# cwchenwang/outdoor-nerf-depth

Hardware: AMD Instinct MI355X
Metric: train rays/sec, KITTI 375x1242, 64+128 samples/ray (higher is better)
Workload: dtype bf16 MFMA operands, f32 accumulate / f32 master weights

## Files before the change

include/nerfpp_hip.h:

```cpp
#ifndef NERFPP_HIP_H
#define NERFPP_HIP_H

#include <stdint.h>

#ifdef __cplusplus
extern "C" {
#endif

#define NERFPP_ABI_VERSION 9

#define NERFPP_OK 0
#define NERFPP_ERR_ARG 1
#define NERFPP_ERR_HIP 2
#define NERFPP_ERR_INTERNAL 3
#define NERFPP_ERR_UNSUPPORTED 4
#define NERFPP_ERR_COMM 5
#define NERFPP_ERR_LAUNCH NERFPP_ERR_HIP

#define NERFPP_PREC_BF16 1
#define NERFPP_PREC_SPLIT_BF16 2
#define NERFPP_PREC_FP16X2W 3

#define NERFPP_LOSS_RGB_ONLY 0
#define NERFPP_LOSS_MSE 1
#define NERFPP_LOSS_L1 2
#define NERFPP_LOSS_KL 3

#define NERFPP_FG_PARAMS 595844
#define NERFPP_BG_PARAMS 606596
#define NERFPP_LEVEL_PARAMS 1202440
#define NERFPP_MAX_SAMPLES 256

const char* nerfpp_last_error(void);
int nerfpp_abi_version(void);


int nerfpp_intersect_sphere(void* stream, int n_rays, const float* ray_o, const float* ray_d,
                            float* fg_far, int* bad_count);

int nerfpp_sample_coarse(void* stream, int n_rays, int n_samples, const float* ray_o,
                         const float* ray_d, const float* min_depth, const float* t_rand_fg,
                         const float* t_rand_bg, float* fg_far, float* fg_z, float* bg_z,
                         int* bad_count);

int nerfpp_sample_coarse_rng(void* stream, int n_rays, int n_samples, const float* ray_o,
                             const float* ray_d, const float* min_depth, uint64_t seed, uint64_t step,
                             float* fg_far, float* fg_z, float* bg_z, int* bad_count);

int nerfpp_rng_uniform(void* stream, uint64_t seed, uint64_t step, int stream_id, int64_t n, float* out);

int nerfpp_perturb_samples(void* stream, int n_rays, int n_samples, const float* z_vals,
                           const float* t_rand, float* out);

int nerfpp_sample_pdf(void* stream, int n_rays, int n_bins_m, int n_new, const float* bins,
                      const float* weights, const float* u, float* samples, int64_t* above_inds);

int nerfpp_sample_fine(void* stream, int n_rays, int s_old, int n_new, const float* z_old,
                       const float* weights, const float* u, float* z_merged, float* samples,
                       int64_t* above_inds);

int nerfpp_sample_fine_pair(void* stream, int n_rays, int s_old, int n_new, const float* fg_z_old,
                            const float* fg_weights, const float* fg_u, float* fg_z_merged,
                            const float* bg_z_old, const float* bg_weights, const float* bg_u,
                            float* bg_z_merged);

int nerfpp_sample_fine_pair_rng(void* stream, int n_rays, int s_old, int n_new, const float* fg_z_old,
                                const float* fg_weights, float* fg_z_merged, const float* bg_z_old,
                                const float* bg_weights, float* bg_z_merged, uint64_t seed, uint64_t step);

int nerfpp_sample_pixels(void* stream, uint64_t seed, uint64_t step, int64_t n_pixels, int n_rays, int64_t* pix);

int nerfpp_gather_rays(void* stream, int n_rays, int width, const float* cam, const int64_t* pix,
                       const float* rgb_img, const float* depth_img, float* ray_o, float* ray_d,
                       float* rgb, float* depth_sup, float* min_depth);


int nerfpp_table_sizes(int net, int64_t* fwd_elems, int64_t* fwd_bias_elems, int64_t* bwd_elems,
                       int64_t* slab_floats, int64_t* n_params);
int nerfpp_build_tables(int net, int32_t* fwd_tbl, int32_t* bias_tbl, int32_t* bwd_tbl,
                        int32_t* unpack_tbl);
int64_t nerfpp_level_tables_elems(void);
int nerfpp_build_level_tables(int32_t* host_tables);

int nerfpp_dw_plan(int64_t rows, int backward_precision, int32_t* k_out, int32_t* is_full_out);

int64_t nerfpp_packed_bytes(int precision);
int nerfpp_pack_level(void* stream, int precision, const float* params, const int32_t* tables,
                      void* packed);


int64_t nerfpp_workspace_bytes(int n_rays, int n_samples, int precision, int training);

int nerfpp_workspace_tensor(int n_rays, int n_samples, int precision, int net, int tensor,
                            int64_t* byte_offset, int32_t* ld, int64_t* plane_bytes);

typedef struct {
  int32_t n_rays, n_samples;
  int32_t precision, training;
  const float* ray_o;
  const float* ray_d;
  const float* fg_far;
  const float* fg_z;
  const float* bg_z;
  const void* packed;
  void* workspace;
  float* rgb;
  float* depth;
  float* fg_weights;
  float* bg_weights;
  float* fg_dists;
  float* fg_rgb;
  float* fg_depth;
  float* bg_rgb;
  float* bg_depth;
  float* bg_lambda;
  void* ev_mlp_begin;
  void* ev_mlp_end;
} nerfpp_forward_args;

int nerfpp_level_forward(void* stream, const nerfpp_forward_args* args);

int nerfpp_loss(void* stream, int n_rays, int n_samples, int loss_type, float lambda_depth,
                float kl_sigma, const float* rgb, const float* rgb_gt, const float* depth,
                const float* depth_sup, const float* fg_weights, const float* fg_z,
                const float* fg_dists, const float* fg_far, float* scalars, float* g_rgb,
                float* g_depth, float* g_fg_weights);

typedef struct {
  int32_t n_rays, n_samples;
  int32_t precision;
  int32_t workspace_precision;
  const float* ray_d;
  const float* fg_far;
  const float* fg_z;
  const float* bg_z;
  const void* packed;
  void* workspace;
  const int32_t* tables;
  const float* g_rgb;
  const float* g_depth;
  const float* g_fg_weights;
  float grad_scale;
  float* grads;
  void* ev_bwd_begin;
  void* ev_bwd_end;
  void* ev_dw_begin;
  void* ev_dw_end;
  const float* params;
  int32_t defer_reduce;
  int32_t fused_loss;
  int32_t loss_type;
  float lambda_depth;
  float kl_sigma;
  const float* rgb;
  const float* depth;
  const float* rgb_gt;
  const float* depth_sup;
  const int32_t* bad_count;
} nerfpp_backward_args;

int nerfpp_level_backward(void* stream, const nerfpp_backward_args* args);

int nerfpp_level_reduce_grads(void* stream, const nerfpp_backward_args* args);

int nerfpp_adam_step(void* stream, float* params, const float* grads, float* exp_avg,
                     float* exp_avg_sq, int64_t n, int step, double lr, double beta1, double beta2,
                     double eps, const float* skip_if_nonzero);

const char* nerfpp_comm_last_error(void);
int nerfpp_rccl_unique_id(char out_id[128]);
int nerfpp_rccl_comm_init(void** comm, int world_size, const char id[128], int rank);
int nerfpp_rccl_comm_destroy(void* comm);
int nerfpp_allreduce_mean(void* stream, void* rccl_comm, float* grads, int64_t count, int world_size, int prescaled);

int64_t nerfpp_image_metrics_workspace_bytes(int n_frames, int H, int W);
int nerfpp_image_metrics_u8(void* stream, int n_frames, int H, int W, const uint8_t* gt, const uint8_t* pred,
                            void* workspace, double* out);

#ifdef __cplusplus
}
#endif
#endif
```

outdoor_nerf_depth_amd/_lib.py:

```python
import ctypes as C
import os

from . import _ctypes_util as U

_HERE = os.path.dirname(os.path.abspath(__file__))
LIB_PATH = os.environ.get('NERFPP_HIP_LIB') or os.path.join(_HERE, 'libnerfpp_hip.so')

OK = 0
ABI_VERSION = 9
PREC_BF16, PREC_SPLIT_BF16 = 1, 2
PREC_FP16_FWD = 3
PREC_SPLIT_FWD = 12
LOSS_RGB_ONLY, LOSS_MSE, LOSS_L1, LOSS_KL = 0, 1, 2, 3
LOSS_TYPES = {'rgbonly': LOSS_RGB_ONLY, 'mse': LOSS_MSE, 'l1': LOSS_L1, 'kl': LOSS_KL}
FG_PARAMS, BG_PARAMS, LEVEL_PARAMS = 595844, 606596, 1202440
MAX_SAMPLES = 256

_fp = C.c_void_p
_i64p = C.POINTER(C.c_int64)
_i32p = C.POINTER(C.c_int32)


class ForwardArgs(C.Structure):
    _fields_ = [('n_rays', C.c_int32), ('n_samples', C.c_int32), ('precision', C.c_int32),
                ('training', C.c_int32)] + \
               [(k, _fp) for k in ('ray_o', 'ray_d', 'fg_far', 'fg_z', 'bg_z', 'packed', 'workspace',
                                   'rgb', 'depth', 'fg_weights', 'bg_weights', 'fg_dists', 'fg_rgb',
                                   'fg_depth', 'bg_rgb', 'bg_depth', 'bg_lambda', 'ev_mlp_begin',
                                   'ev_mlp_end')]


class BackwardArgs(C.Structure):
    _fields_ = [('n_rays', C.c_int32), ('n_samples', C.c_int32), ('precision', C.c_int32),
                ('workspace_precision', C.c_int32)] + \
               [(k, _fp) for k in ('ray_d', 'fg_far', 'fg_z', 'bg_z', 'packed', 'workspace', 'tables',
                                   'g_rgb', 'g_depth', 'g_fg_weights')] + \
               [('grad_scale', C.c_float), ('grads', _fp)] + \
               [(k, _fp) for k in ('ev_bwd_begin', 'ev_bwd_end', 'ev_dw_begin', 'ev_dw_end', 'params')] + \
               [('defer_reduce', C.c_int32), ('fused_loss', C.c_int32), ('loss_type', C.c_int32),
                ('lambda_depth', C.c_float), ('kl_sigma', C.c_float)] + \
               [(k, _fp) for k in ('rgb', 'depth', 'rgb_gt', 'depth_sup', 'bad_count')]


SYMBOLS = {
    'nerfpp_last_error': (C.c_char_p, []),
    'nerfpp_abi_version': (C.c_int, []),
    'nerfpp_intersect_sphere': (C.c_int, [_fp, C.c_int, _fp, _fp, _fp, _fp]),
    'nerfpp_sample_coarse': (C.c_int, [_fp, C.c_int, C.c_int] + [_fp] * 9),
    'nerfpp_sample_coarse_rng': (C.c_int, [_fp, C.c_int, C.c_int, _fp, _fp, _fp, C.c_uint64, C.c_uint64, _fp, _fp, _fp, _fp]),
    'nerfpp_rng_uniform': (C.c_int, [_fp, C.c_uint64, C.c_uint64, C.c_int, C.c_int64, _fp]),
    'nerfpp_sample_pixels': (C.c_int, [_fp, C.c_uint64, C.c_uint64, C.c_int64, C.c_int, _fp]),
    'nerfpp_perturb_samples': (C.c_int, [_fp, C.c_int, C.c_int, _fp, _fp, _fp]),
    'nerfpp_sample_pdf': (C.c_int, [_fp, C.c_int, C.c_int, C.c_int, _fp, _fp, _fp, _fp, _fp]),
    'nerfpp_sample_fine': (C.c_int, [_fp, C.c_int, C.c_int, C.c_int, _fp, _fp, _fp, _fp, _fp, _fp]),
    'nerfpp_sample_fine_pair': (C.c_int, [_fp, C.c_int, C.c_int, C.c_int, _fp, _fp, _fp, _fp, _fp, _fp, _fp, _fp]),
    'nerfpp_sample_fine_pair_rng': (C.c_int, [_fp, C.c_int, C.c_int, C.c_int, _fp, _fp, _fp, _fp, _fp, _fp, C.c_uint64,
                                              C.c_uint64]),
    'nerfpp_gather_rays': (C.c_int, [_fp, C.c_int, C.c_int] + [_fp] * 9),
    'nerfpp_table_sizes': (C.c_int, [C.c_int, _i64p, _i64p, _i64p, _i64p, _i64p]),
    'nerfpp_build_tables': (C.c_int, [C.c_int, _i32p, _i32p, _i32p, _i32p]),
    'nerfpp_level_tables_elems': (C.c_int64, []),
    'nerfpp_build_level_tables': (C.c_int, [_i32p]),
    'nerfpp_dw_plan': (C.c_int, [C.c_int64, C.c_int, _i32p, _i32p]),
    'nerfpp_packed_bytes': (C.c_int64, [C.c_int]),
    'nerfpp_pack_level': (C.c_int, [_fp, C.c_int, _fp, _fp, _fp]),
    'nerfpp_workspace_bytes': (C.c_int64, [C.c_int, C.c_int, C.c_int, C.c_int]),
    'nerfpp_workspace_tensor': (C.c_int, [C.c_int, C.c_int, C.c_int, C.c_int, C.c_int, _i64p, _i32p, _i64p]),
    'nerfpp_level_forward': (C.c_int, [_fp, C.POINTER(ForwardArgs)]),
    'nerfpp_loss': (C.c_int, [_fp, C.c_int, C.c_int, C.c_int, C.c_float, C.c_float] + [_fp] * 12),
    'nerfpp_level_backward': (C.c_int, [_fp, C.POINTER(BackwardArgs)]),
    'nerfpp_level_reduce_grads': (C.c_int, [_fp, C.POINTER(BackwardArgs)]),
    'nerfpp_adam_step': (C.c_int, [_fp, _fp, _fp, _fp, _fp, C.c_int64, C.c_int, C.c_double, C.c_double,
                                   C.c_double, C.c_double, _fp]),
    'nerfpp_image_metrics_workspace_bytes': (C.c_int64, [C.c_int, C.c_int, C.c_int]),
    'nerfpp_image_metrics_u8': (C.c_int, [_fp, C.c_int, C.c_int, C.c_int, _fp, _fp, _fp, _fp]),
    'nerfpp_comm_last_error': (C.c_char_p, []),
    'nerfpp_rccl_unique_id': (C.c_int, [C.c_char_p]),
    'nerfpp_rccl_comm_init': (C.c_int, [C.POINTER(C.c_void_p), C.c_int, C.c_char_p, C.c_int]),
    'nerfpp_rccl_comm_destroy': (C.c_int, [_fp]),
    'nerfpp_allreduce_mean': (C.c_int, [_fp, _fp, _fp, C.c_int64, C.c_int, C.c_int]),
}

_lib = None


class NerfppError(RuntimeError):
    pass


def lib():
    global _lib
    if _lib is None:
        _lib = U.load(LIB_PATH, 'libnerfpp_hip.so', SYMBOLS, 'nerfpp_abi_version', ABI_VERSION, NerfppError,
                      ' (hipcc --offload-arch=gfx950). There is no CPU fallback for the NeRF++ hot path.')
    return _lib


check = U.checker(lib, 'nerfpp_last_error', NerfppError, 'nerfpp call')


def build_level_tables():
    import numpy as np
    n = lib().nerfpp_level_tables_elems()
    out = np.empty(n, np.int32)
    check(lib().nerfpp_build_level_tables(out.ctypes.data_as(_i32p)), 'nerfpp_build_level_tables')
    return out


def build_net_tables(net):
    import numpy as np
    sizes = [C.c_int64() for _ in range(5)]
    check(lib().nerfpp_table_sizes(net, *[C.byref(s) for s in sizes]), 'nerfpp_table_sizes')
    fwd, bias, bwd, slab, npar = [s.value for s in sizes]
    arrs = [np.empty(n, np.int32) for n in (fwd, bias, bwd, npar)]
    check(lib().nerfpp_build_tables(net, *[a.ctypes.data_as(_i32p) for a in arrs]), 'nerfpp_build_tables')
    return arrs[0], arrs[1], arrs[2], arrs[3], slab
```

outdoor_nerf_depth_amd/csrc/nerfpp_api.hip:

```cpp
#include "probe_env.h"
#include <hip/hip_runtime.h>
#include <stdio.h>
#include <stdlib.h>
#include <string.h>
#include "../../include/nerfpp_hip.h"
#define API_OK NERFPP_OK
#define API_ERR_HIP NERFPP_ERR_HIP
#define API_ERR_ARG NERFPP_ERR_ARG
#include "api_common.h"
#include "nerfpp_common.h"
#include "nerfpp_kernels.h"

using namespace nerfpp;

namespace {

constexpr size_t align_up(size_t v, size_t a) { return (v + a - 1) / a * a; }
bool h0_recomputed(int WP) { return a_planes(WP) == 1; }

struct TblLayout { int64_t fwd[2], bias[2], bwd[2], unpack[2], total; };
TblLayout tbl_layout() {
  TblLayout L{};
  int64_t off = 0;
  for (int net = 0; net < N_NET; ++net) {
    L.fwd[net] = off; off += (int64_t)fwd_frags(net) * 512;
    L.bias[net] = off; off += FWD_BIAS_FLOATS;
    L.bwd[net] = off; off += (int64_t)BWD_FRAGS * 512;
    L.unpack[net] = off; off += net_params(net);
  }
  L.total = off;
  return L;
}

struct PackLayout { size_t fwd[2], bwd[2], bias[2], derived[2], total; };
PackLayout pack_layout(int P) {
  PackLayout L{};
  size_t off = 0;
  for (int net = 0; net < N_NET; ++net) {
    L.fwd[net] = off; off = align_up(off + fwd_stream_bytes(net, P), 256);
    L.bwd[net] = off; off = align_up(off + bwd_stream_bytes(P), 256);
    L.bias[net] = off; off = align_up(off + FWD_BIAS_FLOATS * sizeof(float), 256);
    L.derived[net] = off; off = align_up(off + DERIVED_FLOATS * sizeof(float), 256);
  }
  L.total = off;
  return L;
}

struct WsLayout {
  size_t tensor[2][T_COUNT], out_raw[2], depth_real, d_out[2], slabs[2], masks[2], fix_m[2], total;
  int64_t rows, rows_padded;
  int ksplit;
};
int choose_ksplit(int64_t rows) {
  int k = 1;
  for (int rc = 0; rc < 2; ++rc) {
    const DwPlan pl = dw_plan(rows, rc != 0);
    for (int net = 0; net < N_NET; ++net)
      for (int j = 0; j < DW_JOBS; ++j) k = pl.k[net][j] > k ? pl.k[net][j] : k;
  }
  return k;
}
WsLayout ws_layout(int n_rays, int S, int P, bool training) {
  WsLayout L{};
  L.rows = (int64_t)n_rays * S;
  L.rows_padded = (int64_t)align_up((size_t)L.rows, 256);
  L.ksplit = choose_ksplit(L.rows);
  size_t off = 0;
  for (int net = 0; net < N_NET; ++net) {
    L.out_raw[net] = off; off = align_up(off + (size_t)L.rows_padded * 16, 256);
    if (training) {
      L.d_out[net] = off; off = align_up(off + (size_t)L.rows_padded * 16, 256);
      for (int t = 0; t < T_COUNT; ++t) {
        L.tensor[net][t] = off;
        if (t == T_R || t == T_DR) continue;
        if (t == T_DG) continue;
        if (t == T_H0 && h0_recomputed(P)) continue;
        if (t == T_DZ0 + 7 && h0_recomputed(P)) continue;
        off = align_up(off + (size_t)L.rows_padded * tensor_ld(net, t) * 2 * a_planes(P), 256);
      }
      L.slabs[net] = off; off = align_up(off + (size_t)L.ksplit * gslab_floats(net) * 4, 256);
      L.masks[net] = off; off = align_up(off + (size_t)9 * (L.rows_padded / 32) * 64 * 16, 256);
      L.fix_m[net] = off; off = align_up(off + (size_t)128 * 256 * 4, 256);
    }
  }
  L.depth_real = off; off = align_up(off + (size_t)L.rows_padded * 4, 256);
  L.total = off;
  return L;
}

NetWs make_netws(char* ws, const WsLayout& L, int net) {
  NetWs w;
  for (int t = 0; t < T_COUNT; ++t) w.t[t] = (__bf16*)(ws + L.tensor[net][t]);
  w.t[T_DG] = w.t[T_DS] + (DG_COL0 / 16) * (FRAG_BYTES / 2);
  return w;
}

bool prec_ok(int P) { return P == NERFPP_PREC_BF16 || P == NERFPP_PREC_SPLIT_BF16; }
bool prec_ok_fwd(int P) { return prec_ok(P) || P == NERFPP_PREC_FP16X2W; }

bool split_nets() {
  static const bool on = PROBE_GETENV("NERFPP_MLP_SPLIT") != nullptr;
  return on;
}

}

extern "C" {

const char* nerfpp_last_error(void) { return g_err; }
int nerfpp_abi_version(void) { return NERFPP_ABI_VERSION; }

int nerfpp_intersect_sphere(void* stream, int n_rays, const float* ray_o, const float* ray_d, float* fg_far,
                            int* bad_count) {
  REQUIRE(n_rays > 0 && ray_o && ray_d && fg_far, "non-null inputs, n_rays > 0");
  launch_intersect_sphere((hipStream_t)stream, n_rays, ray_o, ray_d, fg_far, bad_count);
  return check_launch("intersect_sphere");
}

int nerfpp_sample_coarse(void* stream, int n_rays, int n_samples, const float* ray_o, const float* ray_d,
                         const float* min_depth, const float* t_rand_fg, const float* t_rand_bg, float* fg_far,
                         float* fg_z, float* bg_z, int* bad_count) {
  REQUIRE(n_rays > 0 && n_samples >= 2 && n_samples <= NERFPP_MAX_SAMPLES, "2 <= n_samples <= 256");
  REQUIRE(ray_o && ray_d && min_depth && fg_far && fg_z && bg_z, "non-null pointers");
  launch_sample_coarse((hipStream_t)stream, n_rays, n_samples, ray_o, ray_d, min_depth, t_rand_fg, t_rand_bg,
                       fg_far, fg_z, bg_z, bad_count, make_rng_key(0, 0, false));
  return check_launch("sample_coarse");
}

int nerfpp_sample_coarse_rng(void* stream, int n_rays, int n_samples, const float* ray_o, const float* ray_d,
                             const float* min_depth, uint64_t seed, uint64_t step, float* fg_far, float* fg_z,
                             float* bg_z, int* bad_count) {
  REQUIRE(n_rays > 0 && n_samples >= 2 && n_samples <= NERFPP_MAX_SAMPLES, "2 <= n_samples <= 256");
  REQUIRE(ray_o && ray_d && min_depth && fg_far && fg_z && bg_z, "non-null pointers");
  launch_sample_coarse((hipStream_t)stream, n_rays, n_samples, ray_o, ray_d, min_depth, nullptr, nullptr, fg_far,
                       fg_z, bg_z, bad_count, make_rng_key(seed, step, true));
  return check_launch("sample_coarse_rng");
}

int nerfpp_rng_uniform(void* stream, uint64_t seed, uint64_t step, int stream_id, int64_t n, float* out) {
  REQUIRE(n > 0 && out && stream_id >= 0 && stream_id <= 3, "stream_id in 0..3, non-null output");
  launch_rng_uniform((hipStream_t)stream, make_rng_key(seed, step, true), (uint32_t)stream_id, n, out);
  return check_launch("rng_uniform");
}

int nerfpp_perturb_samples(void* stream, int n_rays, int n_samples, const float* z_vals, const float* t_rand,
                           float* out) {
  REQUIRE(n_rays > 0 && n_samples >= 2 && z_vals && t_rand && out, "non-null pointers");
  launch_perturb((hipStream_t)stream, n_rays, n_samples, z_vals, t_rand, out);
  return check_launch("perturb_samples");
}

int nerfpp_sample_pdf(void* stream, int n_rays, int n_bins_m, int n_new, const float* bins, const float* weights,
                      const float* u, float* samples, int64_t* above_inds) {
  REQUIRE(n_rays > 0 && n_bins_m >= 1 && n_bins_m + 1 <= 512 && n_new >= 1 && n_new <= 512, "sizes");
  REQUIRE(bins && weights && samples, "non-null pointers");
  launch_sample_pdf((hipStream_t)stream, false, n_rays, n_bins_m, n_new, bins, weights, u, samples, above_inds,
                    nullptr);
  return check_launch("sample_pdf");
}

int nerfpp_sample_fine(void* stream, int n_rays, int s_old, int n_new, const float* z_old, const float* weights,
                       const float* u, float* z_merged, float* samples, int64_t* above_inds) {
  REQUIRE(n_rays > 0 && s_old >= 3 && n_new >= 1 && s_old + n_new <= 512, "3 <= s_old, s_old + n_new <= 512");
  REQUIRE(z_old && weights && z_merged, "non-null pointers");
  launch_sample_pdf((hipStream_t)stream, true, n_rays, s_old - 2, n_new, z_old, weights, u, samples, above_inds,
                    z_merged);
  return check_launch("sample_fine");
}

int nerfpp_sample_fine_pair(void* stream, int n_rays, int s_old, int n_new, const float* fg_z_old,
                            const float* fg_weights, const float* fg_u, float* fg_z_merged, const float* bg_z_old,
                            const float* bg_weights, const float* bg_u, float* bg_z_merged) {
  REQUIRE(n_rays > 0 && s_old >= 3 && n_new >= 1 && s_old + n_new <= 512, "3 <= s_old, s_old + n_new <= 512");
  REQUIRE(fg_z_old && fg_weights && fg_z_merged && bg_z_old && bg_weights && bg_z_merged, "non-null pointers");
  const float* z[2] = {fg_z_old, bg_z_old};
  const float* w[2] = {fg_weights, bg_weights};
  const float* u[2] = {fg_u, bg_u};
  float* m[2] = {fg_z_merged, bg_z_merged};
  launch_sample_fine_pair((hipStream_t)stream, n_rays, s_old - 2, n_new, z, w, u, m, make_rng_key(0, 0, false));
  return check_launch("sample_fine_pair");
}

int nerfpp_sample_fine_pair_rng(void* stream, int n_rays, int s_old, int n_new, const float* fg_z_old,
                                const float* fg_weights, float* fg_z_merged, const float* bg_z_old,
                                const float* bg_weights, float* bg_z_merged, uint64_t seed, uint64_t step) {
  REQUIRE(n_rays > 0 && s_old >= 3 && n_new >= 1 && s_old + n_new <= 512, "3 <= s_old, s_old + n_new <= 512");
  REQUIRE(fg_z_old && fg_weights && fg_z_merged && bg_z_old && bg_weights && bg_z_merged, "non-null pointers");
  const float* z[2] = {fg_z_old, bg_z_old};
  const float* w[2] = {fg_weights, bg_weights};
  const float* u[2] = {nullptr, nullptr};
  float* m[2] = {fg_z_merged, bg_z_merged};
  launch_sample_fine_pair((hipStream_t)stream, n_rays, s_old - 2, n_new, z, w, u, m, make_rng_key(seed, step, true));
  return check_launch("sample_fine_pair_rng");
}

int nerfpp_sample_pixels(void* stream, uint64_t seed, uint64_t step, int64_t n_pixels, int n_rays, int64_t* pix) {
  REQUIRE(pix && n_rays >= 1 && n_rays <= 8192, "1 <= n_rays <= 8192, non-null output");
  REQUIRE(n_pixels >= n_rays && n_pixels < ((int64_t)1 << 31), "n_rays <= n_pixels < 2^31");
  launch_sample_pixels((hipStream_t)stream, make_rng_key(seed, step, true), n_pixels, n_rays, pix);
  return check_launch("sample_pixels");
}

int nerfpp_gather_rays(void* stream, int n_rays, int width, const float* cam, const int64_t* pix,
                       const float* rgb_img, const float* depth_img, float* ray_o, float* ray_d, float* rgb,
                       float* depth_sup, float* min_depth) {
  REQUIRE(n_rays > 0 && width > 0 && cam && pix && ray_o && ray_d && min_depth, "non-null pointers");
  REQUIRE((rgb == nullptr) || rgb_img, "rgb output needs rgb_img");
  REQUIRE((depth_sup == nullptr) || depth_img, "depth_sup output needs depth_img");
  launch_gather_rays((hipStream_t)stream, n_rays, width, cam, pix, rgb_img, depth_img, ray_o, ray_d, rgb, depth_sup,
                     min_depth);
  return check_launch("gather_rays");
}

int64_t nerfpp_level_tables_elems(void) { return tbl_layout().total; }

int nerfpp_build_level_tables(int32_t* host_tables) {
  if (!host_tables) return fail(NERFPP_ERR_ARG, "nerfpp_build_level_tables: null buffer");
  const TblLayout L = tbl_layout();
  for (int net = 0; net < N_NET; ++net) {
    const int rc = nerfpp_build_tables(net, host_tables + L.fwd[net], host_tables + L.bias[net],
                                       host_tables + L.bwd[net], host_tables + L.unpack[net]);
    if (rc != NERFPP_OK) return fail(rc, "nerfpp_build_tables(%d) failed", net);
  }
  return NERFPP_OK;
}

int nerfpp_dw_plan(int64_t rows, int backward_precision, int32_t* k_out, int32_t* is_full_out) {
  if (!k_out || rows <= 0 || !prec_ok(backward_precision)) return -1;
  const DwPlan pl = dw_plan(rows, backward_precision == 1);
  const JobTable jt = build_all_jobs();
  for (int net = 0; net < N_NET; ++net)
    for (int j = 0; j < DW_JOBS; ++j) {
      k_out[net * DW_JOBS + j] = pl.k[net][j];
      if (is_full_out) is_full_out[net * DW_JOBS + j] = dw_job_is_full(jt.jobs[net][j]) ? 1 : 0;
    }
  return DW_JOBS;
}

int64_t nerfpp_packed_bytes(int precision) { return prec_ok_fwd(precision) ? (int64_t)pack_layout(precision).total : -1; }

int nerfpp_pack_level(void* stream, int precision, const float* params, const int32_t* tables, void* packed) {
  REQUIRE(prec_ok_fwd(precision), "precision must be 1, 2 or 3");
  REQUIRE(params && tables && packed, "non-null pointers");
  const TblLayout T = tbl_layout();
  const PackLayout L = pack_layout(precision);
  hipStream_t st = (hipStream_t)stream;
  char* out = (char*)packed;
  const int32_t* tbl[3 * N_NET];
  void* outs[3 * N_NET];
  int64_t n[3 * N_NET];
  for (int net = 0; net < N_NET; ++net) {
    tbl[3 * net] = tables + T.fwd[net];      outs[3 * net] = out + L.fwd[net];      n[3 * net] = (int64_t)fwd_frags(net) * 512;
    tbl[3 * net + 1] = tables + T.bwd[net];  outs[3 * net + 1] = out + L.bwd[net];  n[3 * net + 1] = (int64_t)BWD_FRAGS * 512;
    tbl[3 * net + 2] = tables + T.bias[net]; outs[3 * net + 2] = out + L.bias[net]; n[3 * net + 2] = FWD_BIAS_FLOATS;
  }
  float* derived[N_NET] = {(float*)(out + L.derived[0]), (float*)(out + L.derived[1])};
  launch_pack_level(st, params, precision, tbl, outs, n, derived);
  return check_launch("pack_level");
}

int64_t nerfpp_workspace_bytes(int n_rays, int n_samples, int precision, int training) {
  if (n_rays <= 0 || n_samples < 2 || n_samples > NERFPP_MAX_SAMPLES || !prec_ok_fwd(precision)) return -1;
  return (int64_t)ws_layout(n_rays, n_samples, precision, training != 0).total;
}

int nerfpp_workspace_tensor(int n_rays, int n_samples, int precision, int net, int tensor, int64_t* byte_offset,
                            int32_t* ld, int64_t* plane_bytes) {
  REQUIRE(n_rays > 0 && n_samples >= 2 && n_samples <= NERFPP_MAX_SAMPLES && prec_ok_fwd(precision), "sizes / precision");
  REQUIRE(net >= 0 && net < N_NET && tensor >= 0 && tensor < T_COUNT && tensor != T_R && tensor != T_DR, "net / tensor id");
  REQUIRE(byte_offset && ld && plane_bytes, "non-null outputs");
  if (tensor == T_H0 && h0_recomputed(precision))
    return fail(NERFPP_ERR_UNSUPPORTED, "nerfpp_workspace_tensor: H0 is not materialised at precision %d (its weight-gradient job recomputes it from X)", precision);
  if (tensor == T_DZ0 + 7 && h0_recomputed(precision))
    return fail(NERFPP_ERR_UNSUPPORTED, "nerfpp_workspace_tensor: dZ7 is not materialised at precision %d (its weight-gradient job recomputes it from [dS | dG])", precision);
  const WsLayout L = ws_layout(n_rays, n_samples, precision, true);
  const int l = tensor_ld(net, tensor);
  *byte_offset = tensor == T_DG ? (int64_t)L.tensor[net][T_DS] + (DG_COL0 / 16) * FRAG_BYTES : (int64_t)L.tensor[net][tensor];
  *ld = l;
  *plane_bytes = (int64_t)L.rows_padded * l * 2;
  return NERFPP_OK;
}

int nerfpp_level_forward(void* stream, const nerfpp_forward_args* a) {
  REQUIRE(a, "args");
  REQUIRE(a->n_rays > 0 && a->n_samples >= 2 && a->n_samples <= NERFPP_MAX_SAMPLES, "sizes");
  REQUIRE(prec_ok_fwd(a->precision), "precision must be 1, 2 or 3");
  REQUIRE(a->ray_o && a->ray_d && a->fg_far && a->fg_z && a->bg_z && a->packed && a->workspace, "inputs");
  REQUIRE(a->rgb && a->depth && a->fg_weights && a->bg_weights && a->fg_dists && a->fg_rgb && a->fg_depth &&
          a->bg_rgb && a->bg_depth && a->bg_lambda, "outputs");
  hipStream_t st = (hipStream_t)stream;
  const int P = a->precision;
  const bool train = a->training != 0;
  const WsLayout L = ws_layout(a->n_rays, a->n_samples, P, train);
  const PackLayout PL = pack_layout(P);
  char* ws = (char*)a->workspace;
  const char* pk = (const char*)a->packed;
  MlpFwdArgs mm[N_NET];
  for (int net = 0; net < N_NET; ++net) {
    MlpFwdArgs& m = mm[net];
    m = MlpFwdArgs{};
    m.geom.ray_o = a->ray_o;
    m.geom.ray_d = a->ray_d;
    m.geom.z = net == 0 ? a->fg_z : a->bg_z;
    m.rows = L.rows;
    m.rows_padded = L.rows_padded;
    m.S = a->n_samples;
    m.w_stream = pk + PL.fwd[net];
    m.bias = (const float*)(pk + PL.bias[net]);
    m.out_raw = (float*)(ws + L.out_raw[net]);
    m.depth_real = (float*)(ws + L.depth_real);
    if (train) { m.ws = make_netws(ws, L, net); m.masks = (uint4*)(ws + L.masks[net]); }
    m.save_lo = a->training == 2 ? 0 : 1;
    m.skip_h0 = (train && (h0_recomputed(P) || a->training == 2)) ? 1 : 0;
    if (const char* e = PROBE_GETENV("NERFPP_SKIP_H_RT")) m.save_lo |= atoi(e) << 8;
  }
  if (a->ev_mlp_begin) (void)hipEventRecord((hipEvent_t)a->ev_mlp_begin, st);
  if (split_nets()) {
    launch_mlp_fwd_pair(st, P, train, mm[0], mm[1], 1);
    launch_mlp_fwd_pair(st, P, train, mm[0], mm[1], 2);
  } else {
    launch_mlp_fwd_pair(st, P, train, mm[0], mm[1], 0);
  }
  if (a->ev_mlp_end) (void)hipEventRecord((hipEvent_t)a->ev_mlp_end, st);
  launch_composite_fwd(st, a->n_rays, a->n_samples, (const float*)(ws + L.out_raw[0]),
                       (const float*)(ws + L.out_raw[1]), (const float*)(ws + L.depth_real), a->ray_d, a->fg_far,
                       a->fg_z, a->bg_z, a->rgb, a->depth, a->fg_weights, a->bg_weights, a->fg_dists, a->fg_rgb,
                       a->fg_depth, a->bg_rgb, a->bg_depth, a->bg_lambda);
  return check_launch("level_forward");
}

int nerfpp_loss(void* stream, int n_rays, int n_samples, int loss_type, float lambda_depth, float kl_sigma,
                const float* rgb, const float* rgb_gt, const float* depth, const float* depth_sup,
                const float* fg_weights, const float* fg_z, const float* fg_dists, const float* fg_far,
                float* scalars, float* g_rgb, float* g_depth, float* g_fg_weights) {
  REQUIRE(n_rays > 0 && loss_type >= 0 && loss_type <= 3, "loss_type in 0..3");
  REQUIRE(rgb && rgb_gt && scalars && g_rgb && g_depth, "non-null pointers");
  if (loss_type != NERFPP_LOSS_RGB_ONLY) REQUIRE(depth && depth_sup, "depth loss needs depth and depth_sup");
  if (loss_type == NERFPP_LOSS_KL)
    REQUIRE(fg_weights && fg_z && fg_dists && fg_far && g_fg_weights && kl_sigma > 0.f, "KL inputs");
  launch_loss((hipStream_t)stream, n_rays, n_samples, loss_type, lambda_depth, kl_sigma, rgb, rgb_gt, depth,
              depth_sup, fg_weights, fg_z, fg_dists, fg_far, scalars, g_rgb, g_depth, g_fg_weights);
  return check_launch("loss");
}

}

static void weight_grads(hipStream_t st, const nerfpp_backward_args* a, const WsLayout& L) {
  char* ws = (char*)a->workspace;
  DwArgs dw{};
  for (int net = 0; net < N_NET; ++net) {
    dw.ws[net] = make_netws(ws, L, net);
    dw.slabs[net] = (float*)(ws + L.slabs[net]);
  }
  dw.rows = L.rows;
  dw.rows_padded = L.rows_padded;
  dw.h0_from_x = a->precision == 1 ? 1 : 0;
  const PackLayout PL = pack_layout(a->precision);
  for (int net = 0; net < N_NET; ++net) {
    dw.fwd_w[net] = (const char*)a->packed + PL.fwd[net];
    dw.fwd_bias[net] = (const float*)((const char*)a->packed + PL.bias[net]);
    dw.bwd_w[net] = (const char*)a->packed + PL.bwd[net];
    dw.masks[net] = (const uint4*)(ws + L.masks[net]);
  }
  dw.plan = dw_plan(L.rows, dw.h0_from_x != 0);
  if (a->ev_dw_begin) (void)hipEventRecord((hipEvent_t)a->ev_dw_begin, st);
  launch_dw(st, a->precision, dw);
  if (a->ev_dw_end) (void)hipEventRecord((hipEvent_t)a->ev_dw_end, st);
}
static bool defer_dw() {
  static const bool on = PROBE_GETENV("NERFPP_DEFER_DW") != nullptr;
  return on;
}

static void reduce_grads(hipStream_t st, const nerfpp_backward_args* a, const WsLayout& L, const TblLayout& T) {
  char* ws = (char*)a->workspace;
  const DwPlan plan = dw_plan(L.rows, a->precision == 1);
  const float* slabs[N_NET];
  int64_t slab_floats[N_NET];
  const int32_t* utbl[N_NET];
  float* m_out[N_NET];
  for (int net = 0; net < N_NET; ++net) {
    slabs[net] = (const float*)(ws + L.slabs[net]);
    slab_floats[net] = gslab_floats(net);
    utbl[net] = a->tables + T.unpack[net];
    m_out[net] = (float*)(ws + L.fix_m[net]);
  }
  static const int skip = PROBE_GETENV("NERFPP_REDUCE_SKIP") ? atoi(PROBE_GETENV("NERFPP_REDUCE_SKIP")) : 0;
  if (!(skip & 1)) launch_unpack_grads(st, slabs, slab_floats, plan, utbl, m_out, a->grad_scale, a->grads, a->bad_count);
  if (!(skip & 2)) launch_remap_fixup(st, a->grads, a->params, m_out[0], m_out[1]);
}

extern "C" {

int nerfpp_level_reduce_grads(void* stream, const nerfpp_backward_args* a) {
  REQUIRE(a, "args");
  REQUIRE(a->n_rays > 0 && a->n_samples >= 2 && a->n_samples <= NERFPP_MAX_SAMPLES, "sizes");
  REQUIRE(prec_ok(a->precision), "precision must be 1 or 2");
  REQUIRE(a->workspace && a->tables && a->grads && a->params, "workspace / tables / grads / params");
  const int WP = a->workspace_precision ? a->workspace_precision : a->precision;
  REQUIRE(prec_ok_fwd(WP) && a_planes(WP) >= a_planes(a->precision), "workspace_precision: 0, or a forward precision that saved the planes this backward reads");
  const WsLayout L = ws_layout(a->n_rays, a->n_samples, WP, true);
  if (defer_dw()) weight_grads((hipStream_t)stream, a, L);
  reduce_grads((hipStream_t)stream, a, L, tbl_layout());
  return check_launch("level_reduce_grads");
}

int nerfpp_level_backward(void* stream, const nerfpp_backward_args* a) {
  REQUIRE(a, "args");
  REQUIRE(a->n_rays > 0 && a->n_samples >= 2 && a->n_samples <= NERFPP_MAX_SAMPLES, "sizes");
  REQUIRE(prec_ok(a->precision), "precision must be 1 or 2");
  REQUIRE(a->ray_d && a->fg_far && a->fg_z && a->bg_z && a->packed && a->workspace && a->tables, "inputs");
  REQUIRE(a->grads && a->params, "gradients / params");
  LossFuse lf{};
  if (a->fused_loss) {
    REQUIRE(a->loss_type >= NERFPP_LOSS_RGB_ONLY && a->loss_type <= NERFPP_LOSS_KL, "loss_type in 0..3");
    REQUIRE(a->rgb && a->rgb_gt, "fused loss head needs rgb and rgb_gt");
    if (a->loss_type != NERFPP_LOSS_RGB_ONLY) REQUIRE(a->depth && a->depth_sup, "fused depth loss needs depth and depth_sup");
    if (a->loss_type == NERFPP_LOSS_KL) REQUIRE(a->kl_sigma > 0.f, "kl_sigma > 0");
    lf.type = a->loss_type; lf.lambda_depth = a->lambda_depth; lf.kl_sigma = a->kl_sigma;
    lf.rgb = a->rgb; lf.depth = a->depth; lf.rgb_gt = a->rgb_gt; lf.depth_sup = a->depth_sup;
  } else {
    REQUIRE(a->g_rgb && a->g_depth, "dL/d rgb and dL/d depth (or fused_loss)");
  }
  hipStream_t st = (hipStream_t)stream;
  const int P = a->precision;
  const int WP = a->workspace_precision ? a->workspace_precision : P;
  REQUIRE(prec_ok_fwd(WP) && a_planes(WP) >= a_planes(P), "workspace_precision: 0, or a forward precision that saved the planes this backward reads");
  const WsLayout L = ws_layout(a->n_rays, a->n_samples, WP, true);
  const PackLayout PL = pack_layout(P);
  const TblLayout T = tbl_layout();
  char* ws = (char*)a->workspace;
  const char* pk = (const char*)a->packed;
  launch_composite_bwd(st, a->n_rays, a->n_samples, (const float*)(ws + L.out_raw[0]),
                       (const float*)(ws + L.out_raw[1]), (const float*)(ws + L.depth_real), a->ray_d, a->fg_far,
                       a->fg_z, a->bg_z, a->g_rgb, a->g_depth, a->g_fg_weights, (float*)(ws + L.d_out[0]),
                       (float*)(ws + L.d_out[1]), a->fused_loss ? &lf : nullptr);
  MlpBwdArgs mb[N_NET];
  for (int net = 0; net < N_NET; ++net) {
    MlpBwdArgs& m = mb[net];
    m = MlpBwdArgs{};
    m.rows = L.rows;
    m.rows_padded = L.rows_padded;
    m.w_stream = pk + PL.bwd[net];
    m.d_out = (const float*)(ws + L.d_out[net]);
    m.ws = make_netws(ws, L, net);
    m.masks = (const uint4*)(ws + L.masks[net]);
    m.skip_dz7 = P == 1 ? 1 : 0;
  }
  if (a->ev_bwd_begin) (void)hipEventRecord((hipEvent_t)a->ev_bwd_begin, st);
  if (split_nets()) {
    launch_mlp_bwd_pair(st, P, mb[0], mb[1], 1);
    launch_mlp_bwd_pair(st, P, mb[0], mb[1], 2);
  } else {
    launch_mlp_bwd_pair(st, P, mb[0], mb[1], 0);
  }
  if (a->ev_bwd_end) (void)hipEventRecord((hipEvent_t)a->ev_bwd_end, st);
  if (!(a->defer_reduce && defer_dw())) weight_grads(st, a, L);
  if (!a->defer_reduce) reduce_grads(st, a, L, T);
  return check_launch("level_backward");
}

int nerfpp_adam_step(void* stream, float* params, const float* grads, float* exp_avg, float* exp_avg_sq,
                     int64_t n, int step, double lr, double beta1, double beta2, double eps,
                     const float* skip_if_nonzero) {
  REQUIRE(params && grads && exp_avg && exp_avg_sq && n > 0 && step >= 1, "non-null pointers, step >= 1");
  launch_adam((hipStream_t)stream, params, grads, exp_avg, exp_avg_sq, n, step, lr, beta1, beta2, eps, skip_if_nonzero);
  return check_launch("adam_step");
}

static int image_metrics_sizes_ok(const char* fn, int n_frames, int H, int W) {
  if (n_frames < 1 || n_frames > 65535) return fail(NERFPP_ERR_ARG, "%s: n_frames = %d, expected 1 .. 65535", fn, n_frames);
  if (H < 7 || W < 7)
    return fail(NERFPP_ERR_ARG, "%s: a %d x %d image is smaller than the 7 x 7 SSIM window (H >= 7 and W >= 7)", fn, H, W);
  if (H > 32768 || W > 32768) return fail(NERFPP_ERR_ARG, "%s: a %d x %d image exceeds 32768 pixels per side", fn, H, W);
  return NERFPP_OK;
}

int64_t nerfpp_image_metrics_workspace_bytes(int n_frames, int H, int W) {
  if (image_metrics_sizes_ok(__func__, n_frames, H, W) != NERFPP_OK) return -1;
  return (int64_t)n_frames * image_metrics_tiles(H, W) * 4 * 8;
}

int nerfpp_image_metrics_u8(void* stream, int n_frames, int H, int W, const uint8_t* gt, const uint8_t* pred,
                            void* workspace, double* out) {
  const int rc = image_metrics_sizes_ok(__func__, n_frames, H, W);
  if (rc != NERFPP_OK) return rc;
  REQUIRE(gt && pred && workspace && out, "non-null gt, pred, workspace, out");
  REQUIRE(((uintptr_t)workspace & 7) == 0 && ((uintptr_t)out & 7) == 0, "workspace and out aligned to 8 bytes");
  launch_image_metrics((hipStream_t)stream, n_frames, H, W, gt, pred, workspace, out);
  return check_launch("image_metrics_u8");
}

}
```

outdoor_nerf_depth_amd/csrc/nerfpp_kernels.h:

```cpp
#pragma once
#include <hip/hip_runtime.h>
#include <stdint.h>
#include "nerfpp_common.h"

namespace nerfpp {

struct MlpGeom {
  const float* ray_o;
  const float* ray_d;
  const float* z;
};

struct NetWs {
  __bf16* t[T_COUNT];
};

struct MlpFwdArgs {
  MlpGeom geom;
  int64_t rows, rows_padded;
  int S;
  const void* w_stream;
  const float* bias;
  float* out_raw;
  float* depth_real;
  NetWs ws;
  uint4* masks;
  int save_lo;
  int skip_h0;
};

struct MlpBwdArgs {
  int64_t rows, rows_padded;
  const void* w_stream;
  const float* d_out;
  NetWs ws;
  const uint4* masks;
  int skip_dz7;
};

struct LossFuse {
  int type;
  float lambda_depth, kl_sigma;
  const float* rgb;
  const float* depth;
  const float* rgb_gt;
  const float* depth_sup;
};

struct DwArgs {
  NetWs ws[N_NET];
  int64_t rows, rows_padded;
  float* slabs[N_NET];
  DwPlan plan;
  int h0_from_x;
  const void* fwd_w[N_NET];
  const float* fwd_bias[N_NET];
  const void* bwd_w[N_NET];
  const uint4* masks[N_NET];
};

}

void launch_intersect_sphere(hipStream_t st, int n, const float* o, const float* d, float* far, int* bad);
void launch_sample_coarse(hipStream_t st, int n, int S, const float* o, const float* d, const float* min_depth,
                          const float* t_fg, const float* t_bg, float* far, float* fg_z, float* bg_z, int* bad,
                          const nerfpp::RngKey& rng);
void launch_rng_uniform(hipStream_t st, const nerfpp::RngKey& rng, uint32_t stream_id, int64_t n, float* out);
void launch_perturb(hipStream_t st, int n, int S, const float* z, const float* t, float* out);
void launch_sample_pdf(hipStream_t st, bool fused, int n, int M, int S_new, const float* bins_or_zold,
                       const float* weights, const float* u, float* samples, int64_t* above, float* merged);
void launch_sample_fine_pair(hipStream_t st, int n, int M, int S_new, const float* const* z_old,
                             const float* const* weights, const float* const* u, float* const* merged,
                             const nerfpp::RngKey& rng);
void launch_composite_fwd(hipStream_t st, int n, int S, const float* raw_fg, const float* raw_bg,
                          const float* depth_real_bg, const float* ray_d, const float* fg_far,
                          const float* fg_z, const float* bg_z, float* rgb, float* depth, float* fg_weights,
                          float* bg_weights, float* fg_dists, float* fg_rgb, float* fg_depth, float* bg_rgb,
                          float* bg_depth, float* bg_lambda);
void launch_composite_bwd(hipStream_t st, int n, int S, const float* raw_fg, const float* raw_bg,
                          const float* depth_real_bg, const float* ray_d, const float* fg_far,
                          const float* fg_z, const float* bg_z, const float* g_rgb, const float* g_depth,
                          const float* g_fg_weights, float* dout_fg, float* dout_bg, const nerfpp::LossFuse* lf);
void launch_loss(hipStream_t st, int n, int S, int type, float lambda_depth, float kl_sigma, const float* rgb,
                 const float* rgb_gt, const float* depth, const float* depth_sup, const float* fg_weights,
                 const float* fg_z, const float* fg_dists, const float* fg_far, float* scalars, float* g_rgb,
                 float* g_depth, float* g_fg_weights);
int launch_sample_pixels(hipStream_t st, const nerfpp::RngKey& rng, int64_t n_pixels, int k, int64_t* pix);
void launch_gather_rays(hipStream_t st, int n, int W, const float* cam, const int64_t* pix, const float* rgb_img,
                        const float* depth_img, float* ray_o, float* ray_d, float* rgb, float* depth_sup,
                        float* min_depth);
void launch_mlp_fwd_pair(hipStream_t st, int P, bool train, const nerfpp::MlpFwdArgs& a_fg, const nerfpp::MlpFwdArgs& a_bg, int which);
void launch_mlp_bwd_pair(hipStream_t st, int P, const nerfpp::MlpBwdArgs& a_fg, const nerfpp::MlpBwdArgs& a_bg, int which);
void launch_dw(hipStream_t st, int P, const nerfpp::DwArgs& a);
void launch_pack_level(hipStream_t st, const float* params, int P, const int32_t* const* tbl, void* const* out,
                       const int64_t* n, float* const* derived);
void launch_unpack_grads(hipStream_t st, const float* const* slabs, const int64_t* slab_floats,
                         const nerfpp::DwPlan& plan, const int32_t* const* tbl, float* const* m_out, float scale,
                         float* grads_lvl, const int32_t* bad_count);
void launch_remap_fixup(hipStream_t st, float* grads_lvl, const float* params_lvl, const float* m0, const float* m1);
void launch_adam(hipStream_t st, float* p, const float* g, float* m, float* v, int64_t n, int step, double lr,
                 double beta1, double beta2, double eps, const float* skip);
int64_t image_metrics_tiles(int H, int W);
void launch_image_metrics(hipStream_t st, int F, int H, int W, const unsigned char* gt, const unsigned char* pred,
                          void* workspace, double* out);
```

outdoor_nerf_depth_amd/csrc/nerfpp_render.hip:

```cpp
#include <hip/hip_runtime.h>
#include <math.h>
#include <stdint.h>
#include "hip_device.h"
#include "nerfpp_common.h"
#include "nerfpp_kernels.h"

namespace nerfpp {

using hipdev::wave_sum, hipdev::wave_excl_suffix_sum;

constexpr float TINY = 1e-6f;
constexpr float HUGE_NUM = 1e10f;

__device__ __forceinline__ float sum3(float a, float b, float c) { return (a + b) + c; }

__device__ __forceinline__ float sphere_far(const float* __restrict__ ray_o,
                                            const float* __restrict__ ray_d, int ray, int* bad) {
  const float ox = ray_o[ray * 3], oy = ray_o[ray * 3 + 1], oz = ray_o[ray * 3 + 2];
  const float dx = ray_d[ray * 3], dy = ray_d[ray * 3 + 1], dz = ray_d[ray * 3 + 2];
  const float dd = sum3(dx * dx, dy * dy, dz * dz);
  const float d1 = -sum3(dx * ox, dy * oy, dz * oz) / dd;
  const float px = ox + d1 * dx, py = oy + d1 * dy, pz = oz + d1 * dz;
  const float ray_d_cos = 1.f / sqrtf(dd);
  const float pn = sum3(px * px, py * py, pz * pz);
  if (pn >= 1.f && bad) atomicAdd(bad, 1);
  const float d2 = sqrtf(1.f - pn) * ray_d_cos;
  return d1 + d2;
}

__global__ void intersect_sphere_kernel(int n, const float* __restrict__ ray_o,
                                        const float* __restrict__ ray_d, float* __restrict__ far,
                                        int* bad) {
  const int ray = blockIdx.x * blockDim.x + threadIdx.x;
  if (ray < n) far[ray] = sphere_far(ray_o, ray_d, ray, bad);
}

__device__ __forceinline__ float torch_linspace01(int i, int steps) {
  const float step = 1.f / (float)(steps - 1);
  return i < steps / 2 ? fmaf(step, (float)i, 0.f) : fmaf(-step, (float)(steps - 1 - i), 1.f);
}

__device__ __forceinline__ float perturb(float zm, float z0, float zp, bool first, bool last, float t) {
  const float upper = last ? z0 : .5f * (zp + z0);
  const float lower = first ? z0 : .5f * (z0 + zm);
  return lower + (upper - lower) * t;
}

__global__ void sample_coarse_kernel(int n, int S, const float* __restrict__ ray_o,
                                     const float* __restrict__ ray_d,
                                     const float* __restrict__ min_depth,
                                     const float* __restrict__ t_fg, const float* __restrict__ t_bg,
                                     float* __restrict__ fg_far, float* __restrict__ fg_z,
                                     float* __restrict__ bg_z, int* bad, RngKey rng) {
  const int idx = blockIdx.x * blockDim.x + threadIdx.x;
  if (idx >= n * S) return;
  const int ray = idx / S, i = idx - ray * S;
  const float far = sphere_far(ray_o, ray_d, ray, i == 0 ? bad : nullptr);
  if (i == 0) fg_far[ray] = far;
  const float near = min_depth[ray];
  const float step = (far - near) / (float)(S - 1);
  const float z0 = near + (float)i * step;
  float out = z0;
  if (t_fg || rng.enabled) {
    const float zm = near + (float)(i - 1) * step, zp = near + (float)(i + 1) * step;
    out = perturb(zm, z0, zp, i == 0, i == S - 1, rng.enabled ? philox_uniform(rng, 0, (uint64_t)idx) : t_fg[idx]);
  }
  fg_z[idx] = out;
  const float b0 = torch_linspace01(i, S);
  out = b0;
  if (t_bg || rng.enabled) {
    const float bm = i > 0 ? torch_linspace01(i - 1, S) : 0.f;
    const float bp = i < S - 1 ? torch_linspace01(i + 1, S) : 0.f;
    out = perturb(bm, b0, bp, i == 0, i == S - 1, rng.enabled ? philox_uniform(rng, 1, (uint64_t)idx) : t_bg[idx]);
  }
  bg_z[idx] = out;
}

__global__ void rng_uniform_kernel(RngKey rng, uint32_t stream_id, int64_t n, float* __restrict__ out) {
  const int64_t i = (int64_t)blockIdx.x * blockDim.x + threadIdx.x;
  if (i < n) out[i] = philox_uniform(rng, stream_id, (uint64_t)i);
}

__global__ void perturb_kernel(int n, int S, const float* __restrict__ z, const float* __restrict__ t,
                               float* __restrict__ out) {
  const int idx = blockIdx.x * blockDim.x + threadIdx.x;
  if (idx >= n * S) return;
  const int i = idx % S;
  const float z0 = z[idx];
  const float zm = i > 0 ? z[idx - 1] : 0.f, zp = i < S - 1 ? z[idx + 1] : 0.f;
  out[idx] = perturb(zm, z0, zp, i == 0, i == S - 1, t[idx]);
}

constexpr int SP_MAX = 512;
__device__ __forceinline__ void lds_wave_sync() {
  asm volatile("s_waitcnt lgkmcnt(0)" ::: "memory");
  __builtin_amdgcn_wave_barrier();
}

struct SamplePdfProblem {
  const float* bins_or_zold; const float* weights; const float* u;
  float* samples; int64_t* above; float* merged;
};
struct SamplePdfArgs { SamplePdfProblem p[2]; RngKey rng; };
template <bool FUSED>
__global__ __launch_bounds__(256) void sample_pdf_kernel(int n, int M, int S_new, SamplePdfArgs args) {
  const SamplePdfProblem& pr = args.p[blockIdx.y];
  const float* __restrict__ bins_or_zold = pr.bins_or_zold;
  const float* __restrict__ weights = pr.weights;
  const float* __restrict__ u_in = pr.u;
  float* __restrict__ samples_out = pr.samples;
  int64_t* __restrict__ above_out = pr.above;
  float* __restrict__ merged_out = pr.merged;
  __shared__ float s_cdf[4][SP_MAX];
  __shared__ float s_w[4][SP_MAX];
  __shared__ float s_bins[4][SP_MAX];
  __shared__ float s_z[4][SP_MAX];
  const int wave = threadIdx.x >> 6, lane = threadIdx.x & 63;
  const int ray = blockIdx.x * 4 + wave;
  const bool active = ray < n;
  const int S_old = FUSED ? M + 2 : 0;
  float* cdf = s_cdf[wave];
  float* wq = s_w[wave];
  float* bins = s_bins[wave];
  float* zs = s_z[wave];
  if (active) {
    if (FUSED) {
      const float* zo = bins_or_zold + (size_t)ray * S_old;
      for (int i = lane; i < S_old; i += 64) zs[i] = zo[i];
      for (int k = lane; k < M; k += 64) wq[k] = weights[(size_t)ray * S_old + k + 1] + TINY;
    } else {
      for (int i = lane; i <= M; i += 64) bins[i] = bins_or_zold[(size_t)ray * (M + 1) + i];
      for (int k = lane; k < M; k += 64) wq[k] = weights[(size_t)ray * M + k] + TINY;
    }
  }
  __syncthreads();
  if (active) {
    if (FUSED)
      for (int i = lane; i <= M; i += 64) bins[i] = .5f * (zs[i + 1] + zs[i]);
    if (lane == 0) {
      double acc = 0.0;
      for (int k = 0; k < M; ++k) acc += (double)wq[k];
      cdf[0] = (float)acc;
    }
  }
  __syncthreads();
  if (active) {
    const float wsum = cdf[0];
    for (int k = lane; k < M; k += 64) wq[k] = wq[k] / wsum;
  }
  __syncthreads();
  if (active && lane == 0) {
    double acc = 0.0;
    cdf[0] = 0.f;
    for (int k = 0; k < M; ++k) {
      acc += (double)wq[k];
      cdf[k + 1] = (float)acc;
    }
  }
  __syncthreads();
  if (active) {
    for (int j = lane; j < S_new; j += 64) {
      const float u = args.rng.enabled ? philox_uniform(args.rng, 2u + blockIdx.y, (uint64_t)ray * S_new + j)
                      : u_in ? u_in[(size_t)ray * S_new + j] : torch_linspace01(j, S_new);
      int above = 0, hi_ = M;
      while (above < hi_) {
        const int mid = (above + hi_) >> 1;
        const bool ge = u >= cdf[mid];
        above = ge ? mid + 1 : above;
        hi_ = ge ? hi_ : mid;
      }
      const int below = above - 1 > 0 ? above - 1 : 0;
      const float cdf_lo = cdf[below], cdf_hi = cdf[above];
      const float bin_lo = bins[below], bin_hi = bins[above];
      float denom = cdf_hi - cdf_lo;
      denom = denom < TINY ? 1.f : denom;
      const float t = (u - cdf_lo) / denom;
      const float s = bin_lo + t * (bin_hi - bin_lo + TINY);
      if (samples_out) samples_out[(size_t)ray * S_new + j] = s;
      if (above_out) above_out[(size_t)ray * S_new + j] = above;
      if (FUSED) zs[S_old + j] = s;
    }
  }
  if (!FUSED) return;
  __syncthreads();
  if (active && merged_out) {
    const int S_tot = S_old + S_new;
    bool sorted_old = true;
    for (int i = lane; i + 1 < S_old; i += 64) sorted_old = sorted_old && zs[i] <= zs[i + 1];
    if (__all(sorted_old) && S_new <= SP_MAX) {
      int P2 = 1;
      while (P2 < S_new) P2 <<= 1;
      float* nb = wq;
      for (int i = lane; i < P2; i += 64) nb[i] = i < S_new ? zs[S_old + i] : __builtin_inff();
      lds_wave_sync();
      for (int k = 2; k <= P2; k <<= 1) {
        for (int j = k >> 1; j > 0; j >>= 1) {
          for (int t = lane; t < (P2 >> 1); t += 64) {
            const int lo = ((t & ~(j - 1)) << 1) | (t & (j - 1)), hi_i = lo | j;
            const bool up = (lo & k) == 0;
            const float x = nb[lo], y = nb[hi_i];
            if ((x > y) == up) { nb[lo] = y; nb[hi_i] = x; }
          }
          lds_wave_sync();
        }
      }
      float* mo = merged_out + (size_t)ray * S_tot;
      for (int i = lane; i < S_old; i += 64) {
        const float v = zs[i];
        int lo = 0, hi_i = S_new;
        while (lo < hi_i) {
          const int mid = (lo + hi_i) >> 1;
          const bool lt = nb[mid] < v;
          lo = lt ? mid + 1 : lo;
          hi_i = lt ? hi_i : mid;
        }
        mo[i + lo] = v;
      }
      for (int p = lane; p < S_new; p += 64) {
        const float v = nb[p];
        int lo = 0, hi_i = S_old;
        while (lo < hi_i) {
          const int mid = (lo + hi_i) >> 1;
          const bool le = zs[mid] <= v;
          lo = le ? mid + 1 : lo;
          hi_i = le ? hi_i : mid;
        }
        mo[p + lo] = v;
      }
      return;
    }
    if (S_tot <= 192) {
      const int e0 = lane, e1 = lane + 64, e2 = lane + 128;
      const float v0 = e0 < S_tot ? zs[e0] : 0.f, v1 = e1 < S_tot ? zs[e1] : 0.f, v2 = e2 < S_tot ? zs[e2] : 0.f;
      int r0 = 0, r1 = 0, r2 = 0;
#pragma unroll 4
      for (int k = 0; k < S_tot; ++k) {
        const float o = zs[k];
        r0 += (o < v0 || (o == v0 && k < e0)) ? 1 : 0;
        r1 += (o < v1 || (o == v1 && k < e1)) ? 1 : 0;
        r2 += (o < v2 || (o == v2 && k < e2)) ? 1 : 0;
      }
      float* mo = merged_out + (size_t)ray * S_tot;
      if (e0 < S_tot) mo[r0] = v0;
      if (e1 < S_tot) mo[r1] = v1;
      if (e2 < S_tot) mo[r2] = v2;
      return;
    }
    for (int e = lane; e < S_tot; e += 64) {
      const float v = zs[e];
      int rank = 0;
      for (int k = 0; k < S_tot; ++k) {
        const float o = zs[k];
        rank += (o < v || (o == v && k < e)) ? 1 : 0;
      }
      merged_out[(size_t)ray * S_tot + rank] = v;
    }
  }
}

constexpr int CPL_MAX = 4;

__device__ __forceinline__ float wave_excl_prod(float x, int lane, float* total) {
  float v = x;
#pragma unroll
  for (int d = 1; d < 64; d <<= 1) {
    const float t = __shfl_up(v, d, 64);
    if (lane >= d) v *= t;
  }
  *total = __shfl(v, 63, 64);
  const float e = __shfl_up(v, 1, 64);
  return lane == 0 ? 1.f : e;
}

struct RaySamples {
  float dist[CPL_MAX], e[CPL_MAX], alpha[CPL_MAX], q[CPL_MAX], T[CPL_MAX], w[CPL_MAX];
  float c[CPL_MAX][3], zval[CPL_MAX], sraw[CPL_MAX];
  float lambda;
};

template <bool BG>
__device__ __forceinline__ void load_volume(RaySamples& v, int S, int cpl, int lane, size_t row0,
                                            const float4* __restrict__ raw, const float* __restrict__ z,
                                            const float* __restrict__ depth_real, float dnorm, float far) {
  float run = 1.f;
#pragma unroll
  for (int k = 0; k < CPL_MAX; ++k) {
    const int i = lane * cpl + k;
    const bool ok = k < cpl && i < S;
    float dist = 0.f, sraw = 0.f, zv = 0.f;
    float c0 = 0.f, c1 = 0.f, c2 = 0.f;
    if (ok) {
      const int s = BG ? S - 1 - i : i;
      const float4 r = raw[row0 + s];
      c0 = r.x; c1 = r.y; c2 = r.z; sraw = r.w;
      if (BG) {
        const float zi = z[s];
        dist = i < S - 1 ? zi - z[s - 1] : HUGE_NUM;
        zv = depth_real[row0 + s];
      } else {
        const float zi = z[i];
        dist = dnorm * ((i < S - 1 ? z[i + 1] : far) - zi);
        zv = zi;
      }
    }
    const float sigma = fabsf(sraw);
    const float e = ok ? expf(-sigma * dist) : 1.f;
    const float alpha = 1.f - e;
    const float q = ok ? 1.f - alpha + TINY : 1.f;
    v.dist[k] = dist; v.e[k] = e; v.alpha[k] = alpha; v.q[k] = q;
    v.c[k][0] = c0; v.c[k][1] = c1; v.c[k][2] = c2; v.zval[k] = zv; v.sraw[k] = sraw;
    v.T[k] = run;
    run *= q;
  }
  float total;
  const float pre = wave_excl_prod(run, lane, &total);
  v.lambda = total;
#pragma unroll
  for (int k = 0; k < CPL_MAX; ++k) {
    v.T[k] *= pre;
    v.w[k] = v.alpha[k] * v.T[k];
  }
}

__global__ __launch_bounds__(256) void composite_fwd_kernel(
    int n, int S, const float4* __restrict__ raw_fg, const float4* __restrict__ raw_bg,
    const float* __restrict__ depth_real_bg, const float* __restrict__ ray_d,
    const float* __restrict__ fg_far, const float* __restrict__ fg_z, const float* __restrict__ bg_z,
    float* __restrict__ rgb, float* __restrict__ depth, float* __restrict__ fg_weights,
    float* __restrict__ bg_weights, float* __restrict__ fg_dists, float* __restrict__ fg_rgb,
    float* __restrict__ fg_depth, float* __restrict__ bg_rgb, float* __restrict__ bg_depth,
    float* __restrict__ bg_lambda) {
  const int wave = threadIdx.x >> 6, lane = threadIdx.x & 63;
  const int ray = blockIdx.x * 4 + wave;
  if (ray >= n) return;
  const int cpl = (S + 63) / 64;
  const size_t row0 = (size_t)ray * S;
  const float dx = ray_d[ray * 3], dy = ray_d[ray * 3 + 1], dz = ray_d[ray * 3 + 2];
  const float dnorm = sqrtf(sum3(dx * dx, dy * dy, dz * dz));
  RaySamples v;
  load_volume<false>(v, S, cpl, lane, row0, raw_fg, fg_z + row0, nullptr, dnorm, fg_far[ray]);
  float a0 = 0, a1 = 0, a2 = 0, ad = 0;
#pragma unroll
  for (int k = 0; k < CPL_MAX; ++k) {
    const int i = lane * cpl + k;
    if (k < cpl && i < S) {
      fg_weights[row0 + i] = v.w[k];
      fg_dists[row0 + i] = v.dist[k];
      a0 += v.w[k] * v.c[k][0]; a1 += v.w[k] * v.c[k][1]; a2 += v.w[k] * v.c[k][2];
      ad += v.w[k] * v.zval[k];
    }
  }
  const float f0 = wave_sum(a0), f1 = wave_sum(a1), f2 = wave_sum(a2), fd = wave_sum(ad);
  const float lam = v.lambda;
  load_volume<true>(v, S, cpl, lane, row0, raw_bg, bg_z + row0, depth_real_bg, dnorm, 0.f);
  a0 = a1 = a2 = ad = 0;
#pragma unroll
  for (int k = 0; k < CPL_MAX; ++k) {
    const int i = lane * cpl + k;
    if (k < cpl && i < S) {
      bg_weights[row0 + i] = v.w[k];
      a0 += v.w[k] * v.c[k][0]; a1 += v.w[k] * v.c[k][1]; a2 += v.w[k] * v.c[k][2];
      ad += v.w[k] * v.zval[k];
    }
  }
  const float b0 = lam * wave_sum(a0), b1 = lam * wave_sum(a1), b2 = lam * wave_sum(a2);
  const float bd = lam * wave_sum(ad);
  if (lane == 0) {
    fg_rgb[ray * 3] = f0; fg_rgb[ray * 3 + 1] = f1; fg_rgb[ray * 3 + 2] = f2;
    bg_rgb[ray * 3] = b0; bg_rgb[ray * 3 + 1] = b1; bg_rgb[ray * 3 + 2] = b2;
    rgb[ray * 3] = f0 + b0; rgb[ray * 3 + 1] = f1 + b1; rgb[ray * 3 + 2] = f2 + b2;
    fg_depth[ray] = fd; bg_depth[ray] = bd; depth[ray] = fd + bd; bg_lambda[ray] = lam;
  }
}

struct KlFuse { bool on; float gt, inv2s, lambda_depth; };
template <bool BG>
__device__ __forceinline__ void volume_backward(const RaySamples& v, int S, int cpl, int lane, size_t row0,
                                                const float gC[3], float gD, float g_lam_lam,
                                                const float* __restrict__ g_w_extra,
                                                float4* __restrict__ dout, const KlFuse kl = KlFuse{false, 0.f, 0.f, 0.f}) {
  float gw[CPL_MAX], term = 0.f;
#pragma unroll
  for (int k = 0; k < CPL_MAX; ++k) {
    const int i = lane * cpl + k;
    const bool ok = k < cpl && i < S;
    float g = gC[0] * v.c[k][0] + gC[1] * v.c[k][1] + gC[2] * v.c[k][2] + gD * v.zval[k];
    if (ok && g_w_extra) g += g_w_extra[row0 + i];
    if (!BG && ok && kl.on) {
      const float dz = v.zval[k] - kl.gt;
      const float w = v.w[k] + 1e-5f;
      const float e = expf(-(dz * dz) * kl.inv2s);
      g += -kl.lambda_depth * e * v.dist[k] / (w * (float)S);
    }
    gw[k] = ok ? g : 0.f;
    term += gw[k] * v.w[k];
  }
  float suffix = wave_excl_suffix_sum(term, lane);
#pragma unroll
  for (int k = CPL_MAX - 1; k >= 0; --k) {
    const int i = lane * cpl + k;
    if (k < cpl && i < S) {
      const float d_a = gw[k] * v.T[k] - (suffix + g_lam_lam) / v.q[k];
      const float d_sigma = d_a * v.dist[k] * v.e[k];
      const float sgn = v.sraw[k] > 0.f ? 1.f : (v.sraw[k] < 0.f ? -1.f : 0.f);
      float4 o;
      o.x = v.w[k] * gC[0] * v.c[k][0] * (1.f - v.c[k][0]);
      o.y = v.w[k] * gC[1] * v.c[k][1] * (1.f - v.c[k][1]);
      o.z = v.w[k] * gC[2] * v.c[k][2] * (1.f - v.c[k][2]);
      o.w = d_sigma * sgn;
      const int s = BG ? S - 1 - i : i;
      dout[row0 + s] = o;
    }
    suffix += gw[k] * v.w[k];
  }
}

template <bool LF>
__global__ __launch_bounds__(256) void composite_bwd_kernel(
    int n, int S, const float4* __restrict__ raw_fg, const float4* __restrict__ raw_bg,
    const float* __restrict__ depth_real_bg, const float* __restrict__ ray_d,
    const float* __restrict__ fg_far, const float* __restrict__ fg_z, const float* __restrict__ bg_z,
    const float* __restrict__ g_rgb, const float* __restrict__ g_depth,
    const float* __restrict__ g_fg_weights, float4* __restrict__ dout_fg, float4* __restrict__ dout_bg, LossFuse lf) {
  const int wave = threadIdx.x >> 6, lane = threadIdx.x & 63;
  const int ray = blockIdx.x * 4 + wave;
  float cnt = 0.f;
  if (LF && (lf.type == 1 || lf.type == 2)) {
    __shared__ float s_cnt[4];
    float c = 0.f;
    for (int r = threadIdx.x; r < n; r += 256) c += lf.depth_sup[r] > 0.f ? 1.f : 0.f;
    c = wave_sum(c);
    if (lane == 0) s_cnt[wave] = c;
    __syncthreads();
    cnt = (s_cnt[0] + s_cnt[1]) + (s_cnt[2] + s_cnt[3]);
  }
  if (ray >= n) return;
  const int cpl = (S + 63) / 64;
  const size_t row0 = (size_t)ray * S;
  const float dx = ray_d[ray * 3], dy = ray_d[ray * 3 + 1], dz = ray_d[ray * 3 + 2];
  const float dnorm = sqrtf(sum3(dx * dx, dy * dy, dz * dz));
  float gC[3], gD;
  KlFuse kl{false, 0.f, 0.f, 0.f};
  if (LF) {
#pragma unroll
    for (int c = 0; c < 3; ++c) gC[c] = 2.f * (lf.rgb[ray * 3 + c] - lf.rgb_gt[ray * 3 + c]) / (float)(3 * n);
    gD = 0.f;
    if (lf.type == 1 || lf.type == 2) {
      const float gt = lf.depth_sup[ray];
      if (gt > 0.f && cnt > 0.f) {
        const float d = lf.depth[ray] - gt;
        gD = lf.type == 1 ? lf.lambda_depth * 2.f * d / cnt
                          : lf.lambda_depth * (d > 0.f ? 1.f : (d < 0.f ? -1.f : 0.f)) / cnt;
      }
    } else if (lf.type == 3) {
      const float gt = lf.depth_sup[ray];
      kl.on = gt > 0.f && gt < fg_far[ray];
      kl.gt = gt;
      kl.inv2s = 1.f / (2.f * lf.kl_sigma);
      kl.lambda_depth = lf.lambda_depth;
    }
  } else {
    gC[0] = g_rgb[ray * 3]; gC[1] = g_rgb[ray * 3 + 1]; gC[2] = g_rgb[ray * 3 + 2];
    gD = g_depth[ray];
  }
  RaySamples vb;
  load_volume<true>(vb, S, cpl, lane, row0, raw_bg, bg_z + row0, depth_real_bg, dnorm, 0.f);
  float a0 = 0, a1 = 0, a2 = 0, ad = 0;
#pragma unroll
  for (int k = 0; k < CPL_MAX; ++k) {
    a0 += vb.w[k] * vb.c[k][0]; a1 += vb.w[k] * vb.c[k][1]; a2 += vb.w[k] * vb.c[k][2];
    ad += vb.w[k] * vb.zval[k];
  }
  const float g_lam = gC[0] * wave_sum(a0) + gC[1] * wave_sum(a1) + gC[2] * wave_sum(a2) + gD * wave_sum(ad);
  RaySamples vf;
  load_volume<false>(vf, S, cpl, lane, row0, raw_fg, fg_z + row0, nullptr, dnorm, fg_far[ray]);
  const float lam = vf.lambda;
  volume_backward<false>(vf, S, cpl, lane, row0, gC, gD, g_lam * lam, LF ? nullptr : g_fg_weights, dout_fg, kl);
  const float gCb[3] = {lam * gC[0], lam * gC[1], lam * gC[2]};
  volume_backward<true>(vb, S, cpl, lane, row0, gCb, lam * gD, 0.f, nullptr, dout_bg);
}

__device__ double block_sum(double v, double* sh) {
  const int t = threadIdx.x;
  sh[t] = v;
  __syncthreads();
  for (int d = blockDim.x >> 1; d > 0; d >>= 1) {
    if (t < d) sh[t] += sh[t + d];
    __syncthreads();
  }
  const double r = sh[0];
  __syncthreads();
  return r;
}

__global__ __launch_bounds__(256) void kl_terms_kernel(
    int n, int S, float lambda_depth, float kl_sigma, const float* __restrict__ depth_sup,
    const float* __restrict__ fg_weights, const float* __restrict__ fg_z, const float* __restrict__ fg_dists,
    const float* __restrict__ fg_far, float* __restrict__ ray_sum, float* __restrict__ g_fg_weights) {
  const int wave = threadIdx.x >> 6, lane = threadIdx.x & 63;
  const int ray = blockIdx.x * 4 + wave;
  if (ray >= n) return;
  const float gt = depth_sup[ray];
  const bool m = gt > 0.f && gt < fg_far[ray];
  const float inv2s = 1.f / (2.f * kl_sigma);
  double acc = 0.0;
  for (int s = lane; s < S; s += 64) {
    const size_t i = (size_t)ray * S + s;
    float g = 0.f;
    if (m) {
      const float dz = fg_z[i] - gt;
      const float w = fg_weights[i] + 1e-5f;
      const float e = expf(-(dz * dz) * inv2s);
      acc += (double)(-logf(w) * e * fg_dists[i]);
      g = -lambda_depth * e * fg_dists[i] / (w * (float)S);
    }
    g_fg_weights[i] = g;
  }
  acc = wave_sum(acc);
  if (lane == 0) ray_sum[ray] = (float)acc;
}

__global__ __launch_bounds__(1024) void loss_kernel(
    int n, int S, int type, float lambda_depth, float kl_sigma, const float* __restrict__ rgb,
    const float* __restrict__ rgb_gt, const float* __restrict__ depth, const float* __restrict__ depth_sup,
    const float* __restrict__ fg_weights, const float* __restrict__ fg_z, const float* __restrict__ fg_dists,
    const float* __restrict__ fg_far, float* __restrict__ scalars, float* __restrict__ g_rgb,
    float* __restrict__ g_depth, float* __restrict__ g_fg_weights) {
  __shared__ double sh[1024];
  double s_rgb = 0, s_dep = 0, s_cnt = 0;
  for (int r = threadIdx.x; r < n; r += blockDim.x) {
    for (int c = 0; c < 3; ++c) {
      const float d = rgb[r * 3 + c] - rgb_gt[r * 3 + c];
      s_rgb += (double)(d * d);
    }
    if (type == 0) continue;
    const float gt = depth_sup[r];
    if (type == 3) {
      const bool m = gt > 0.f && gt < fg_far[r];
      if (m) {
        s_cnt += 1;
        s_dep += (double)g_depth[r];
      }
    } else if (gt > 0.f) {
      const float d = gt - depth[r];
      s_cnt += 1;
      s_dep += type == 1 ? (double)(d * d) : (double)fabsf(d);
    }
  }
  const double t_rgb = block_sum(s_rgb, sh), t_dep = block_sum(s_dep, sh), t_cnt = block_sum(s_cnt, sh);
  const float rgb_loss = (float)(t_rgb / (3.0 * n));
  float depth_loss = 0.f;
  if (type == 3) depth_loss = (float)(t_dep / S);
  else if (type != 0) depth_loss = (float)(t_dep / t_cnt);
  if (threadIdx.x == 0) {
    scalars[0] = type == 0 ? rgb_loss : rgb_loss + lambda_depth * depth_loss;
    scalars[1] = rgb_loss;
    scalars[2] = depth_loss;
    scalars[3] = (float)t_cnt;
  }
  const float cnt = (float)t_cnt;
  for (int r = threadIdx.x; r < n; r += blockDim.x) {
    for (int c = 0; c < 3; ++c)
      g_rgb[r * 3 + c] = 2.f * (rgb[r * 3 + c] - rgb_gt[r * 3 + c]) / (float)(3 * n);
    float gd = 0.f;
    if (type == 1 || type == 2) {
      const float gt = depth_sup[r];
      if (gt > 0.f && cnt > 0.f) {
        const float d = depth[r] - gt;
        gd = type == 1 ? lambda_depth * 2.f * d / cnt
                       : lambda_depth * (d > 0.f ? 1.f : (d < 0.f ? -1.f : 0.f)) / cnt;
      }
    }
    g_depth[r] = gd;
    if (g_fg_weights && type != 3)
      for (int s = 0; s < S; ++s) g_fg_weights[(size_t)r * S + s] = 0.f;
  }
}

}

using namespace nerfpp;

void launch_intersect_sphere(hipStream_t st, int n, const float* o, const float* d, float* far, int* bad) {
  hipLaunchKernelGGL(intersect_sphere_kernel, dim3((n + 255) / 256), dim3(256), 0, st, n, o, d, far, bad);
}
void launch_sample_coarse(hipStream_t st, int n, int S, const float* o, const float* d, const float* min_depth,
                          const float* t_fg, const float* t_bg, float* far, float* fg_z, float* bg_z, int* bad,
                          const nerfpp::RngKey& rng) {
  const int tot = n * S;
  hipLaunchKernelGGL(sample_coarse_kernel, dim3((tot + 255) / 256), dim3(256), 0, st, n, S, o, d, min_depth,
                     t_fg, t_bg, far, fg_z, bg_z, bad, rng);
}
void launch_rng_uniform(hipStream_t st, const nerfpp::RngKey& rng, uint32_t stream_id, int64_t n, float* out) {
  hipLaunchKernelGGL(rng_uniform_kernel, dim3((unsigned)((n + 255) / 256)), dim3(256), 0, st, rng, stream_id, n, out);
}
void launch_perturb(hipStream_t st, int n, int S, const float* z, const float* t, float* out) {
  const int tot = n * S;
  hipLaunchKernelGGL(perturb_kernel, dim3((tot + 255) / 256), dim3(256), 0, st, n, S, z, t, out);
}
void launch_sample_pdf(hipStream_t st, bool fused, int n, int M, int S_new, const float* bins_or_zold,
                       const float* weights, const float* u, float* samples, int64_t* above, float* merged) {
  dim3 grid((n + 3) / 4), block(256);
  SamplePdfArgs a{};
  a.p[0] = SamplePdfProblem{bins_or_zold, weights, u, samples, above, merged};
  if (fused) hipLaunchKernelGGL(sample_pdf_kernel<true>, grid, block, 0, st, n, M, S_new, a);
  else hipLaunchKernelGGL(sample_pdf_kernel<false>, grid, block, 0, st, n, M, S_new, a);
}
void launch_sample_fine_pair(hipStream_t st, int n, int M, int S_new, const float* const* z_old,
                             const float* const* weights, const float* const* u, float* const* merged,
                             const nerfpp::RngKey& rng) {
  dim3 grid((n + 3) / 4, 2), block(256);
  SamplePdfArgs a{};
  a.rng = rng;
  for (int k = 0; k < 2; ++k) a.p[k] = SamplePdfProblem{z_old[k], weights[k], u[k], nullptr, nullptr, merged[k]};
  hipLaunchKernelGGL(sample_pdf_kernel<true>, grid, block, 0, st, n, M, S_new, a);
}
void launch_composite_fwd(hipStream_t st, int n, int S, const float* raw_fg, const float* raw_bg,
                          const float* depth_real_bg, const float* ray_d, const float* fg_far,
                          const float* fg_z, const float* bg_z, float* rgb, float* depth, float* fg_weights,
                          float* bg_weights, float* fg_dists, float* fg_rgb, float* fg_depth, float* bg_rgb,
                          float* bg_depth, float* bg_lambda) {
  hipLaunchKernelGGL(composite_fwd_kernel, dim3((n + 3) / 4), dim3(256), 0, st, n, S, (const float4*)raw_fg,
                     (const float4*)raw_bg, depth_real_bg, ray_d, fg_far, fg_z, bg_z, rgb, depth, fg_weights,
                     bg_weights, fg_dists, fg_rgb, fg_depth, bg_rgb, bg_depth, bg_lambda);
}
void launch_composite_bwd(hipStream_t st, int n, int S, const float* raw_fg, const float* raw_bg,
                          const float* depth_real_bg, const float* ray_d, const float* fg_far,
                          const float* fg_z, const float* bg_z, const float* g_rgb, const float* g_depth,
                          const float* g_fg_weights, float* dout_fg, float* dout_bg, const nerfpp::LossFuse* lf) {
  if (lf)
    hipLaunchKernelGGL(composite_bwd_kernel<true>, dim3((n + 3) / 4), dim3(256), 0, st, n, S, (const float4*)raw_fg,
                       (const float4*)raw_bg, depth_real_bg, ray_d, fg_far, fg_z, bg_z, g_rgb, g_depth,
                       g_fg_weights, (float4*)dout_fg, (float4*)dout_bg, *lf);
  else
    hipLaunchKernelGGL(composite_bwd_kernel<false>, dim3((n + 3) / 4), dim3(256), 0, st, n, S, (const float4*)raw_fg,
                       (const float4*)raw_bg, depth_real_bg, ray_d, fg_far, fg_z, bg_z, g_rgb, g_depth,
                       g_fg_weights, (float4*)dout_fg, (float4*)dout_bg, nerfpp::LossFuse{});
}
void launch_loss(hipStream_t st, int n, int S, int type, float lambda_depth, float kl_sigma, const float* rgb,
                 const float* rgb_gt, const float* depth, const float* depth_sup, const float* fg_weights,
                 const float* fg_z, const float* fg_dists, const float* fg_far, float* scalars, float* g_rgb,
                 float* g_depth, float* g_fg_weights) {
  if (type == 3)
    hipLaunchKernelGGL(kl_terms_kernel, dim3((n + 3) / 4), dim3(256), 0, st, n, S, lambda_depth, kl_sigma, depth_sup,
                       fg_weights, fg_z, fg_dists, fg_far, g_depth, g_fg_weights);
  hipLaunchKernelGGL(loss_kernel, dim3(1), dim3(1024), 0, st, n, S, type, lambda_depth, kl_sigma, rgb, rgb_gt,
                     depth, depth_sup, fg_weights, fg_z, fg_dists, fg_far, scalars, g_rgb, g_depth,
                     g_fg_weights);
}

namespace nerfpp {
__global__ void gather_rays_kernel(int n, int W, const float* __restrict__ cam, const int64_t* __restrict__ pix,
                                   const float* __restrict__ rgb_img, const float* __restrict__ depth_img,
                                   float* __restrict__ ray_o, float* __restrict__ ray_d, float* __restrict__ rgb,
                                   float* __restrict__ depth_sup, float* __restrict__ min_depth) {
  const int i = blockIdx.x * blockDim.x + threadIdx.x;
  if (i >= n) return;
  const int64_t p = pix[i];
  const float u = (float)(p % W) + 0.5f, v = (float)(p / W) + 0.5f;
  const float cx = (cam[0] * u + cam[1] * v) + cam[2];
  const float cy = (cam[3] * u + cam[4] * v) + cam[5];
  const float cz = (cam[6] * u + cam[7] * v) + cam[8];
  const float* c2w = cam + 9;
  ray_d[i * 3 + 0] = (c2w[0] * cx + c2w[1] * cy) + c2w[2] * cz;
  ray_d[i * 3 + 1] = (c2w[4] * cx + c2w[5] * cy) + c2w[6] * cz;
  ray_d[i * 3 + 2] = (c2w[8] * cx + c2w[9] * cy) + c2w[10] * cz;
  ray_o[i * 3 + 0] = c2w[3]; ray_o[i * 3 + 1] = c2w[7]; ray_o[i * 3 + 2] = c2w[11];
  if (rgb) { rgb[i * 3] = rgb_img[p * 3]; rgb[i * 3 + 1] = rgb_img[p * 3 + 1]; rgb[i * 3 + 2] = rgb_img[p * 3 + 2]; }
  if (depth_sup) depth_sup[i] = depth_img[p];
  min_depth[i] = 1e-4f;
}
}

namespace nerfpp {
constexpr int PIX_THREADS = 1024;
__global__ __launch_bounds__(PIX_THREADS) void sample_pixels_kernel(RngKey rng, uint32_t n, int k, int kp, int64_t* __restrict__ pix) {
  extern __shared__ __attribute__((aligned(16))) char pix_smem[];
  unsigned long long* keys = (unsigned long long*)pix_smem;
  uint32_t* x = (uint32_t*)(pix_smem + (size_t)kp * 8);
  uint32_t* ndraw = x + k;
  __shared__ int again;
  const uint32_t thresh = (0u - n) % n;
  auto draw = [&](int i) {
    uint32_t d = ndraw[i], v;
    for (;;) {
      const uint32_t w = philox_word(rng, 4u, (uint64_t)i + ((uint64_t)d << 20));
      ++d;
      const uint64_t m = (uint64_t)w * n;
      if ((uint32_t)m >= thresh) { v = (uint32_t)(m >> 32); break; }
    }
    ndraw[i] = d;
    x[i] = v;
  };
  for (int i = threadIdx.x; i < k; i += PIX_THREADS) { ndraw[i] = 0; draw(i); }
  for (;;) {
    __syncthreads();
    if (threadIdx.x == 0) again = 0;
    for (int i = threadIdx.x; i < kp; i += PIX_THREADS)
      keys[i] = i < k ? ((unsigned long long)x[i] << 32) | (unsigned)i : ~0ull;
    __syncthreads();
    for (int size = 2; size <= kp; size <<= 1)
      for (int stride = size >> 1; stride > 0; stride >>= 1) {
        for (int t = threadIdx.x; t < kp / 2; t += PIX_THREADS) {
          const int lo = 2 * t - (t & (stride - 1)), hi = lo + stride;
          const bool up = (lo & size) == 0;
          const unsigned long long a = keys[lo], b = keys[hi];
          if ((a > b) == up) { keys[lo] = b; keys[hi] = a; }
        }
        __syncthreads();
      }
    for (int p = threadIdx.x + 1; p < k; p += PIX_THREADS)
      if ((uint32_t)(keys[p] >> 32) == (uint32_t)(keys[p - 1] >> 32)) { draw((int)(uint32_t)keys[p]); again = 1; }
    __syncthreads();
    if (!again) break;
  }
  for (int i = threadIdx.x; i < k; i += PIX_THREADS) pix[i] = (int64_t)x[i];
}
}

int launch_sample_pixels(hipStream_t st, const nerfpp::RngKey& rng, int64_t n_pixels, int k, int64_t* pix) {
  int kp = 2;
  while (kp < k) kp <<= 1;
  const size_t lds = (size_t)kp * 8 + (size_t)k * 8;
  hipLaunchKernelGGL(nerfpp::sample_pixels_kernel, dim3(1), dim3(nerfpp::PIX_THREADS), lds, st, rng, (uint32_t)n_pixels, k, kp, pix);
  return 0;
}

void launch_gather_rays(hipStream_t st, int n, int W, const float* cam, const int64_t* pix, const float* rgb_img,
                        const float* depth_img, float* ray_o, float* ray_d, float* rgb, float* depth_sup,
                        float* min_depth) {
  hipLaunchKernelGGL(nerfpp::gather_rays_kernel, dim3((n + 255) / 256), dim3(256), 0, st, n, W, cam, pix, rgb_img,
                     depth_img, ray_o, ray_d, rgb, depth_sup, min_depth);
}
```

outdoor_nerf_depth_amd/ops.py:

```python
import ctypes as C
import functools
from collections import OrderedDict

import torch

from . import _ctypes_util as U
from . import _lib as L


_stream, _p = U.stream, U.p
_f32 = functools.partial(U.f32, error=L.NerfppError, fallback='the NeRF++ hot path has no CPU fallback')


def intersect_sphere(ray_o, ray_d):
    ray_o, ray_d = _f32(ray_o), _f32(ray_d)
    n = ray_o.shape[0]
    far = torch.empty(n, device=ray_o.device)
    bad = torch.zeros(1, dtype=torch.int32, device=ray_o.device)
    L.check(L.lib().nerfpp_intersect_sphere(_stream(), n, _p(ray_o), _p(ray_d), _p(far), _p(bad)),
            'nerfpp_intersect_sphere')
    if int(bad.item()) != 0:
        raise Exception(CAMERA_ERROR)
    return far


CAMERA_ERROR = ('Not all your cameras are bounded by the unit sphere; please make sure the '
                'cameras are normalized properly!')


def rng_uniform(seed, step, stream_id, shape, device):
    out = torch.empty(shape, device=device)
    L.check(L.lib().nerfpp_rng_uniform(_stream(), int(seed), int(step), int(stream_id), out.numel(), _p(out)),
            'nerfpp_rng_uniform')
    return out


def sample_pixels(n_pixels, n_rays, seed, step, device):
    pix = torch.empty(n_rays, dtype=torch.int64, device=device)
    L.check(L.lib().nerfpp_sample_pixels(_stream(), int(seed), int(step), int(n_pixels), int(n_rays), _p(pix)),
            'nerfpp_sample_pixels')
    return pix


def sample_coarse(ray_o, ray_d, min_depth, n_samples, t_rand_fg=None, t_rand_bg=None, perturb=True,
                  check=True, rng=None, bad=None):
    ray_o, ray_d, min_depth = _f32(ray_o), _f32(ray_d), _f32(min_depth)
    n = ray_o.shape[0]
    dev = ray_o.device
    if rng is not None and perturb:
        far = torch.empty(n, device=dev)
        fg_z = torch.empty(n, n_samples, device=dev)
        bg_z = torch.empty(n, n_samples, device=dev)
        if bad is None:
            bad = torch.zeros(1, dtype=torch.int32, device=dev)
        L.check(L.lib().nerfpp_sample_coarse_rng(_stream(), n, n_samples, _p(ray_o), _p(ray_d), _p(min_depth),
                                                 int(rng[0]), int(rng[1]), _p(far), _p(fg_z), _p(bg_z), _p(bad)),
                'nerfpp_sample_coarse_rng')
        if check and int(bad.item()) != 0:
            raise Exception(CAMERA_ERROR)
        return far, fg_z, bg_z
    if perturb:
        if t_rand_fg is None:
            t_rand_fg = torch.rand(n, n_samples, device=dev)
        if t_rand_bg is None:
            t_rand_bg = torch.rand(n, n_samples, device=dev)
        t_rand_fg, t_rand_bg = _f32(t_rand_fg, (n, n_samples)), _f32(t_rand_bg, (n, n_samples))
    else:
        t_rand_fg = t_rand_bg = None
    far = torch.empty(n, device=dev)
    fg_z = torch.empty(n, n_samples, device=dev)
    bg_z = torch.empty(n, n_samples, device=dev)
    if bad is None:
        bad = torch.zeros(1, dtype=torch.int32, device=dev)
    L.check(L.lib().nerfpp_sample_coarse(_stream(), n, n_samples, _p(ray_o), _p(ray_d), _p(min_depth),
                                         _p(t_rand_fg), _p(t_rand_bg), _p(far), _p(fg_z), _p(bg_z), _p(bad)),
            'nerfpp_sample_coarse')
    if check and int(bad.item()) != 0:
        raise Exception(CAMERA_ERROR)
    return far, fg_z, bg_z


def perturb_samples(z_vals, t_rand=None):
    z_vals = _f32(z_vals)
    if t_rand is None:
        t_rand = torch.rand_like(z_vals)
    t_rand = _f32(t_rand, z_vals.shape)
    out = torch.empty_like(z_vals)
    n, S = z_vals.shape
    L.check(L.lib().nerfpp_perturb_samples(_stream(), n, S, _p(z_vals), _p(t_rand), _p(out)),
            'nerfpp_perturb_samples')
    return out


def sample_pdf(bins, weights, N_samples, det=False, u=None, return_inds=False):
    bins, weights = _f32(bins), _f32(weights)
    n, M = weights.shape
    if bins.shape != (n, M + 1):
        raise L.NerfppError('bins must be [n, M+1]')
    if not det and u is None:
        u = torch.rand(n, N_samples, device=bins.device)
    u = None if det else _f32(u, (n, N_samples))
    samples = torch.empty(n, N_samples, device=bins.device)
    above = torch.empty(n, N_samples, dtype=torch.int64, device=bins.device) if return_inds else None
    L.check(L.lib().nerfpp_sample_pdf(_stream(), n, M, N_samples, _p(bins), _p(weights), _p(u), _p(samples),
                                      _p(above)), 'nerfpp_sample_pdf')
    return (samples, above) if return_inds else samples


def sample_fine(z_old, weights, N_samples, det=False, u=None, return_all=False):
    z_old, weights = _f32(z_old), _f32(weights)
    n, S_old = z_old.shape
    if weights.shape != (n, S_old):
        raise L.NerfppError('weights must be [n, S_old]')
    if not det and u is None:
        u = torch.rand(n, N_samples, device=z_old.device)
    u = None if det else _f32(u, (n, N_samples))
    merged = torch.empty(n, S_old + N_samples, device=z_old.device)
    samples = torch.empty(n, N_samples, device=z_old.device) if return_all else None
    above = torch.empty(n, N_samples, dtype=torch.int64, device=z_old.device) if return_all else None
    L.check(L.lib().nerfpp_sample_fine(_stream(), n, S_old, N_samples, _p(z_old), _p(weights), _p(u), _p(merged),
                                       _p(samples), _p(above)), 'nerfpp_sample_fine')
    return (merged, samples, above) if return_all else merged


def sample_fine_pair(fg_z, fg_weights, bg_z, bg_weights, N_samples, det=False, u_fg=None, u_bg=None, rng=None):
    fg_z, fg_weights, bg_z, bg_weights = _f32(fg_z), _f32(fg_weights), _f32(bg_z), _f32(bg_weights)
    n, S_old = fg_z.shape
    if fg_weights.shape != (n, S_old) or bg_z.shape != (n, S_old) or bg_weights.shape != (n, S_old):
        raise L.NerfppError('z / weights must all be [n, S_old]')
    if rng is not None and not det:
        fg_m = torch.empty(n, S_old + N_samples, device=fg_z.device)
        bg_m = torch.empty(n, S_old + N_samples, device=fg_z.device)
        L.check(L.lib().nerfpp_sample_fine_pair_rng(_stream(), n, S_old, N_samples, _p(fg_z), _p(fg_weights), _p(fg_m),
                                                    _p(bg_z), _p(bg_weights), _p(bg_m), int(rng[0]), int(rng[1])),
                'nerfpp_sample_fine_pair_rng')
        return fg_m, bg_m
    if det:
        u_fg = u_bg = None
    else:
        u_fg = _f32(u_fg, (n, N_samples)) if u_fg is not None else torch.rand(n, N_samples, device=fg_z.device)
        u_bg = _f32(u_bg, (n, N_samples)) if u_bg is not None else torch.rand(n, N_samples, device=fg_z.device)
    fg_m = torch.empty(n, S_old + N_samples, device=fg_z.device)
    bg_m = torch.empty(n, S_old + N_samples, device=fg_z.device)
    L.check(L.lib().nerfpp_sample_fine_pair(_stream(), n, S_old, N_samples, _p(fg_z), _p(fg_weights), _p(u_fg),
                                            _p(fg_m), _p(bg_z), _p(bg_weights), _p(u_bg), _p(bg_m)),
            'nerfpp_sample_fine_pair')
    return fg_m, bg_m


_TABLES = {}


def level_tables(device):
    key = str(device)
    if key not in _TABLES:
        _TABLES[key] = torch.from_numpy(L.build_level_tables()).to(device)
    return _TABLES[key]


RET_KEYS = ('rgb', 'fg_weights', 'bg_weights', 'fg_dists', 'fg_rgb', 'fg_depth', 'bg_rgb', 'bg_depth',
            'bg_lambda', 'depth')


class LevelEngine(object):

    def __init__(self, params_flat, precision=L.PREC_SPLIT_BF16):
        if params_flat.numel() != L.LEVEL_PARAMS:
            raise L.NerfppError('expected %d parameters, got %d' % (L.LEVEL_PARAMS, params_flat.numel()))
        self.params = _f32(params_flat)
        self.device = self.params.device
        precision = int(precision)
        if precision not in (L.PREC_BF16, L.PREC_SPLIT_BF16, L.PREC_FP16_FWD, L.PREC_SPLIT_FWD):
            raise L.NerfppError('unknown precision %r' % (precision,))
        self.precision = L.PREC_SPLIT_BF16 if precision == L.PREC_SPLIT_FWD else precision
        self.bwd_precision = L.PREC_BF16 if precision in (L.PREC_SPLIT_FWD, L.PREC_FP16_FWD) else precision
        self.tables = level_tables(self.device)
        self.packed = torch.empty(L.lib().nerfpp_packed_bytes(self.precision), dtype=torch.uint8,
                                  device=self.device)
        self.packed_bwd = self.packed if self.bwd_precision == self.precision else \
            torch.empty(L.lib().nerfpp_packed_bytes(self.bwd_precision), dtype=torch.uint8, device=self.device)
        self.workspace = None
        self._fwd = None
        self.repack()

    def repack(self):
        L.check(L.lib().nerfpp_pack_level(_stream(), self.precision, _p(self.params), _p(self.tables),
                                          _p(self.packed)), 'nerfpp_pack_level')
        if self.packed_bwd is not self.packed:
            L.check(L.lib().nerfpp_pack_level(_stream(), self.bwd_precision, _p(self.params), _p(self.tables),
                                              _p(self.packed_bwd)), 'nerfpp_pack_level')

    def _workspace(self, n, S, training):
        need = L.lib().nerfpp_workspace_bytes(n, S, self.precision, int(training))
        if need < 0:
            raise L.NerfppError('unsupported sizes n_rays=%d n_samples=%d' % (n, S))
        if self.workspace is None or self.workspace.numel() < need:
            self.workspace = torch.empty(need, dtype=torch.uint8, device=self.device)
        return self.workspace

    def forward(self, ray_o, ray_d, fg_z_max, fg_z_vals, bg_z_vals, training=False, events=None):
        ray_o, ray_d = _f32(ray_o), _f32(ray_d)
        n = ray_o.shape[0]
        fg_z_vals = _f32(fg_z_vals)
        S = fg_z_vals.shape[1]
        bg_z_vals, fg_z_max = _f32(bg_z_vals, (n, S)), _f32(fg_z_max, (n,))
        dev = self.device
        out = OrderedDict()
        for k in RET_KEYS:
            shape = (n, 3) if k in ('rgb', 'fg_rgb', 'bg_rgb') else \
                (n, S) if k in ('fg_weights', 'bg_weights', 'fg_dists') else (n,)
            out[k] = torch.empty(shape, device=dev)
        a = L.ForwardArgs()
        hi_only = training and self.bwd_precision != self.precision
        a.n_rays, a.n_samples, a.precision, a.training = n, S, self.precision, (2 if hi_only else int(training))
        a.ray_o, a.ray_d, a.fg_far, a.fg_z, a.bg_z = [t.data_ptr() for t in
                                                      (ray_o, ray_d, fg_z_max, fg_z_vals, bg_z_vals)]
        a.packed = self.packed.data_ptr()
        a.workspace = self._workspace(n, S, training).data_ptr()
        for k in RET_KEYS:
            setattr(a, k, out[k].data_ptr())
        if events is not None:
            a.ev_mlp_begin, a.ev_mlp_end = events[0].cuda_event, events[1].cuda_event
        L.check(L.lib().nerfpp_level_forward(_stream(), C.byref(a)), 'nerfpp_level_forward')
        if training:
            self._fwd = (n, S, ray_d, fg_z_max, fg_z_vals, bg_z_vals)
        return out

    def saved_tensor(self, net, tensor, plane=0):
        if self._fwd is None:
            raise L.NerfppError('saved_tensor() needs a preceding forward(training=True)')
        n, S = self._fwd[0], self._fwd[1]
        off, ld, pb = C.c_int64(), C.c_int32(), C.c_int64()
        L.check(L.lib().nerfpp_workspace_tensor(n, S, self.precision, int(net), int(tensor), C.byref(off), C.byref(ld),
                                                C.byref(pb)), 'nerfpp_workspace_tensor')
        rows, ld = n * S, ld.value
        rows_p = (rows + 31) // 32 * 32
        nblk = rows_p // 32 * (ld // 16)
        raw = self.workspace[off.value + plane * pb.value: off.value + plane * pb.value + nblk * 1024]
        blk = raw.view(torch.bfloat16).view(rows_p // 32, ld // 16, 32, 2, 8)
        blk = blk.view(rows_p // 32, ld // 16, 32, 2, 2, 4).permute(0, 2, 1, 4, 3, 5)
        return blk.reshape(rows_p, ld)[:rows].float()

    def backward(self, g_rgb, g_depth, g_fg_weights=None, grad_scale=1.0, out=None, events=None, defer_reduce=False,
                 fused_loss=None, bad_count=None):
        if self._fwd is None:
            raise L.NerfppError('backward() needs a preceding forward(training=True)')
        n, S, ray_d, fg_far, fg_z, bg_z = self._fwd
        keep = None
        if fused_loss is None:
            g_rgb, g_depth = _f32(g_rgb, (n, 3)), _f32(g_depth, (n,))
            g_fg_weights = _f32(g_fg_weights, (n, S)) if g_fg_weights is not None else None
        else:
            g_rgb = g_depth = g_fg_weights = None
            f = fused_loss
            t = L.LOSS_TYPES[f['loss_type']]
            keep = (_f32(f['ret']['rgb'], (n, 3)), _f32(f['ret']['depth'], (n,)), _f32(f['rgb_gt'], (n, 3)),
                    _f32(f['depth_sup'], (n,)) if t != L.LOSS_RGB_ONLY else None)
        n_out = L.LEVEL_PARAMS + (1 if bad_count is not None else 0)
        grads = out if out is not None else torch.empty(n_out, device=self.device)
        if grads.numel() < n_out or not grads.is_contiguous() or grads.dtype != torch.float32:
            raise L.NerfppError('backward(): `out` needs %d contiguous float32 elements' % n_out)
        a = L.BackwardArgs()
        a.n_rays, a.n_samples, a.precision = n, S, self.bwd_precision
        a.workspace_precision = self.precision
        a.ray_d, a.fg_far, a.fg_z, a.bg_z = [t.data_ptr() for t in (ray_d, fg_far, fg_z, bg_z)]
        a.packed, a.workspace, a.tables = self.packed_bwd.data_ptr(), self.workspace.data_ptr(), self.tables.data_ptr()
        if fused_loss is None:
            a.g_rgb, a.g_depth = g_rgb.data_ptr(), g_depth.data_ptr()
            a.g_fg_weights = g_fg_weights.data_ptr() if g_fg_weights is not None else None
        else:
            a.fused_loss, a.loss_type = 1, t
            a.lambda_depth, a.kl_sigma = float(fused_loss.get('lambda_depth', 1.0)), float(fused_loss.get('kl_sigma', 0.01))
            a.rgb, a.depth, a.rgb_gt = keep[0].data_ptr(), keep[1].data_ptr(), keep[2].data_ptr()
            a.depth_sup = keep[3].data_ptr() if keep[3] is not None else None
        a.grad_scale = float(grad_scale)
        a.grads = grads.data_ptr()
        a.params = self.params.data_ptr()
        if events is not None:
            a.ev_bwd_begin, a.ev_bwd_end, a.ev_dw_begin, a.ev_dw_end = [e.cuda_event for e in events]
        a.defer_reduce = int(bool(defer_reduce))
        if bad_count is not None:
            if bad_count.dtype != torch.int32 or bad_count.numel() != 1 or bad_count.device != self.device:
                raise L.NerfppError('bad_count: one int32 on the engine\'s device')
            a.bad_count = bad_count.data_ptr()
        L.check(L.lib().nerfpp_level_backward(_stream(), C.byref(a)), 'nerfpp_level_backward')
        self._bwd_args = (a, grads, bad_count, torch.cuda.current_stream()) if defer_reduce else None
        return grads

    def reduce_grads(self):
        if getattr(self, '_bwd_args', None) is None:
            raise L.NerfppError('reduce_grads() needs a preceding backward(defer_reduce=True)')
        a, grads, bad_count, bwd_stream = self._bwd_args
        self._bwd_args = None
        st = torch.cuda.current_stream()
        if bad_count is not None and st != bwd_stream:
            bad_count.record_stream(st)
        L.check(L.lib().nerfpp_level_reduce_grads(_stream(), C.byref(a)), 'nerfpp_level_reduce_grads')
        return grads


def loss_and_grads(ret, rgb_gt, depth_sup=None, loss_type='rgbonly', lambda_depth=1.0, kl_sigma=0.01,
                   fg_z_vals=None, fg_far_depth=None):
    rgb = _f32(ret['rgb'])
    n = rgb.shape[0]
    S = ret['fg_weights'].shape[1]
    dev = rgb.device
    t = L.LOSS_TYPES[loss_type]
    scalars = torch.empty(4, device=dev)
    g_rgb = torch.empty(n, 3, device=dev)
    g_depth = torch.empty(n, device=dev)
    g_w = torch.empty(n, S, device=dev) if t == L.LOSS_KL else None
    rgb_gt = _f32(rgb_gt, (n, 3))
    depth_sup = _f32(depth_sup, (n,)) if depth_sup is not None else None
    fg_z_vals = _f32(fg_z_vals) if fg_z_vals is not None else None
    fg_far_depth = _f32(fg_far_depth) if fg_far_depth is not None else None
    L.check(L.lib().nerfpp_loss(_stream(), n, S, t, float(lambda_depth), float(kl_sigma), _p(rgb), _p(rgb_gt),
                                _p(_f32(ret['depth'])), _p(depth_sup), _p(_f32(ret['fg_weights'])), _p(fg_z_vals),
                                _p(_f32(ret['fg_dists'])), _p(fg_far_depth), _p(scalars), _p(g_rgb), _p(g_depth),
                                _p(g_w)), 'nerfpp_loss')
    return scalars, g_rgb, g_depth, g_w


def adam_step(params, grads, exp_avg, exp_avg_sq, step, lr=5e-4, beta1=0.9, beta2=0.999, eps=1e-8, skip=None):
    if skip is not None and (skip.dtype != torch.float32 or not skip.is_cuda):
        raise L.NerfppError('adam_step: skip must be a float32 device tensor')
    L.check(L.lib().nerfpp_adam_step(_stream(), _p(params), _p(grads), _p(exp_avg), _p(exp_avg_sq),
                                     params.numel(), int(step), lr, beta1, beta2, eps, _p(skip)), 'nerfpp_adam_step')
```

outdoor_nerf_depth_amd/trainer.py:

```python
import os

import numpy as np
import torch

from . import _lib as L
from . import ops
from .model import init_level_params

ALGO_MACS = {
    'fwd': (593408, 604160),
    'dx': (557696, 557696),
}


class NerfppTrainer(object):
    def __init__(self, device, precision=L.PREC_SPLIT_BF16, cascade_samples=(64, 128), lrate=5e-4,
                 use_depth=True, depth_loss_type='mse', lambda_depth=0.1, depth_sigma=0.01, depth_scale=1.0,
                 world_size=1, level_params=None, overlap_allreduce=True, optim_autoexpo=False, img_names=None,
                 lambda_autoexpo=1.0, seed=777, torch_rng=False, fuse_loss=False, comm=None):
        self.device = torch.device(device)
        self.comm = comm
        self.precision = precision
        self.cascade_samples = tuple(cascade_samples)
        self.lrate = lrate
        self.loss_type = depth_loss_type if use_depth else 'rgbonly'
        if self.loss_type not in L.LOSS_TYPES:
            raise ValueError("depth_loss_type %r: only mse / l1 / kl exist in the reference "
                             "('los' and 'nll' are dead code there)" % depth_loss_type)
        self.lambda_depth = lambda_depth
        self.kl_sigma = depth_sigma * depth_scale
        self.world_size = world_size
        if level_params is None:
            level_params = init_level_params(len(self.cascade_samples))
        self.engines = [ops.LevelEngine(p.to(self.device), precision) for p in level_params]
        self.exp_avg = [torch.zeros_like(e.params) for e in self.engines]
        self.exp_avg_sq = [torch.zeros_like(e.params) for e in self.engines]
        self.grads = [torch.zeros(L.LEVEL_PARAMS + 4, device=self.device) for _ in self.engines]
        self.step_count = 0
        self.seed, self.torch_rng = int(seed), bool(torch_rng)
        self.fuse_loss = bool(fuse_loss)
        self.rng_step = 0
        self.bad_cameras = torch.zeros(1, dtype=torch.int32, device=self.device)
        self.autoexpo = None
        if optim_autoexpo:
            if not img_names:
                raise ValueError('optim_autoexpo needs the training image names (ddp_model.py:168)')
            from .autoexpo import AutoExposure
            self.img_names = list(img_names)
            self.autoexpo = [AutoExposure(img_names, self.device, lrate, lambda_autoexpo, world_size)
                             for _ in self.engines]
        self._ae_grad = [None] * len(self.engines)
        self.last_autoexpo = [None] * len(self.engines)
        self.update_stream = torch.cuda.Stream(device=self.device) if overlap_allreduce else None
        self.level_streams = [torch.cuda.Stream(device=self.device) for _ in range(len(self.cascade_samples))] if overlap_allreduce else None
        self.concurrent_backward = True
        self._pending = {}
        self.wait_taps = None
        self.comm_taps = None

    def _update(self, m, step):
        eng = self.engines[m]
        eng.reduce_grads()
        flag = self.grads[m][L.LEVEL_PARAMS:L.LEVEL_PARAMS + 1]
        if self.world_size > 1 or self.comm is not None:
            import torch.distributed as dist
            if self.autoexpo is not None:
                if self._ae_grad[m] is None:
                    self._ae_grad[m] = torch.zeros(len(self.autoexpo[m].names), 3, device=self.device)
                if self.comm is not None:
                    self.comm.allreduce_mean(self._ae_grad[m].view(-1), prescaled=True)
                else:
                    dist.all_reduce(self._ae_grad[m])
            tap = None
            if self.comm_taps is not None:
                tap = (torch.cuda.Event(enable_timing=True), torch.cuda.Event(enable_timing=True))
                tap[0].record()
            if self.comm is not None:
                self.comm.allreduce_mean(self.grads[m], prescaled=True)
            else:
                dist.all_reduce(self.grads[m])
            if tap is not None:
                tap[1].record()
                self.comm_taps.append((m, tap[0], tap[1]))
        ops.adam_step(eng.params, self.grads[m][:L.LEVEL_PARAMS], self.exp_avg[m], self.exp_avg_sq[m], step, lr=self.lrate,
                      skip=flag)
        eng.repack()
        if self._ae_grad[m] is not None:
            self.autoexpo[m].apply(self._ae_grad[m][:, :2], self._ae_grad[m][:, 2] > 0)
            self._ae_grad[m] = None

    def _update_begin(self, m):
        if self.update_stream is None:
            self._update(m, self.step_count)
            return
        ev = torch.cuda.Event()
        ev.record()
        self.update_stream.wait_event(ev)
        if self._ae_grad[m] is not None:
            self._ae_grad[m].record_stream(self.update_stream)
        with torch.cuda.stream(self.update_stream):
            self._update(m, self.step_count)
            done = torch.cuda.Event()
            done.record()
        self._pending[m] = done

    def _update_end(self, m):
        done = self._pending.pop(m, None)
        if done is not None:
            if self.wait_taps is not None:
                a, b = torch.cuda.Event(enable_timing=True), torch.cuda.Event(enable_timing=True)
                a.record()
                torch.cuda.current_stream().wait_event(done)
                b.record()
                self.wait_taps.append((a, b))
            else:
                torch.cuda.current_stream().wait_event(done)

    def flush(self):
        for m in list(self._pending):
            self._update_end(m)

    def check_cameras(self):
        bad = int(self.bad_cameras.item())
        if self.world_size > 1 and self.step_count > 0:
            self.flush()
            bad += int(sum(float(g[L.LEVEL_PARAMS].item()) for g in self.grads))
        if bad != 0:
            self.bad_cameras.zero_()
            for g in self.grads:
                g[L.LEVEL_PARAMS:].zero_()
            raise Exception(ops.CAMERA_ERROR)

    def train_step(self, batch, uniforms=None, events=None):
        self.step_count += 1
        ray_o, ray_d = batch['ray_o'], batch['ray_d']
        n = ray_o.shape[0]
        S0, S1 = self.cascade_samples[0], self.cascade_samples[1] if len(self.cascade_samples) > 1 else 0
        dev = self.device
        u = uniforms or {}
        self.rng_step += 1
        rng = None if (uniforms is not None or self.torch_rng) else (self.seed, self.rng_step)
        if rng is not None:
            far, fg_z, bg_z = ops.sample_coarse(ray_o, ray_d, batch['min_depth'], S0, check=False, rng=rng,
                                                bad=self.bad_cameras)
        else:
            t_fg = u['t_fg'] if 't_fg' in u else torch.rand(n, S0, device=dev)
            t_bg = u['t_bg'] if 't_bg' in u else torch.rand(n, S0, device=dev)
            far, fg_z, bg_z = ops.sample_coarse(ray_o, ray_d, batch['min_depth'], S0, t_fg, t_bg, check=False,
                                                bad=self.bad_cameras)
        depth_sup = batch.get('depth_sup') if self.loss_type != 'rgbonly' else None
        scalars = []
        ret = None
        ae_idx = None
        if self.autoexpo is not None:
            name = batch.get('img_name')
            if name is None and 'frame' in batch:
                name = self.img_names[int(batch['frame'])]
            ae_idx = self.autoexpo[0].lookup(name)
        for m, eng in enumerate(self.engines):
            self._update_end(m)
            if m > 0 and rng is not None:
                fg_z, bg_z = ops.sample_fine_pair(fg_z, ret['fg_weights'], bg_z, ret['bg_weights'], S1, rng=rng)
            elif m > 0:
                u_fg = u['u_fg'] if 'u_fg' in u else torch.rand(n, S1, device=dev)
                u_bg = u['u_bg'] if 'u_bg' in u else torch.rand(n, S1, device=dev)
                fg_z, bg_z = ops.sample_fine_pair(fg_z, ret['fg_weights'], bg_z, ret['bg_weights'], S1,
                                                  u_fg=u_fg, u_bg=u_bg)
            ev = events[m] if events is not None else None
            ret = eng.forward(ray_o, ray_d, far, fg_z, bg_z, training=True,
                              events=ev['fwd'] if ev else None)
            ae = self.autoexpo[m] if ae_idx is not None else None
            if ae is None and self.fuse_loss:
                loss_done = None
                if self.update_stream is not None:
                    fwd_done = torch.cuda.Event()
                    fwd_done.record()
                    self.update_stream.wait_event(fwd_done)
                    with torch.cuda.stream(self.update_stream):
                        sc = ops.loss_and_grads(ret, batch['rgb'], depth_sup, self.loss_type, self.lambda_depth,
                                                self.kl_sigma, fg_z, far)[0]
                        loss_done = torch.cuda.Event()
                        loss_done.record()
                eng.backward(None, None, None, grad_scale=1.0 / self.world_size, out=self.grads[m][:L.LEVEL_PARAMS + 1], bad_count=self.bad_cameras,
                             events=ev['bwd'] if ev else None, defer_reduce=True,
                             fused_loss=dict(loss_type=self.loss_type, lambda_depth=self.lambda_depth, kl_sigma=self.kl_sigma,
                                             ret=ret, rgb_gt=batch['rgb'], depth_sup=depth_sup))
                if loss_done is not None:
                    torch.cuda.current_stream().wait_event(loss_done)
                else:
                    sc = ops.loss_and_grads(ret, batch['rgb'], depth_sup, self.loss_type, self.lambda_depth,
                                            self.kl_sigma, fg_z, far)[0]
                scalars.append(sc)
                self._update_begin(m)
                continue
            rgb_gt = ae.target(ae_idx, batch['rgb']) if ae is not None else batch['rgb']
            sc, g_rgb, g_depth, g_w = ops.loss_and_grads(ret, rgb_gt, depth_sup, self.loss_type,
                                                         self.lambda_depth, self.kl_sigma, fg_z, far)
            if ae is not None:
                g_ae = ae.finish(ae_idx, ret['rgb'], batch['rgb'], sc, g_rgb, self.lambda_depth)
                rows = torch.zeros(len(ae.names), 3, device=dev)
                rows[ae_idx, :2] = g_ae
                rows[ae_idx, 2] = 1.0
                self._ae_grad[m] = rows
                self.last_autoexpo[m] = ae.scale_shift(ae_idx)
            if self.concurrent_backward and m + 1 < len(self.engines) and ae is None and events is None and self.update_stream is not None:
                stream = self.level_streams[m]
                fwd_done = torch.cuda.Event()
                fwd_done.record()
                stream.wait_event(fwd_done)
                for t in [g_rgb, g_depth, g_w, ray_o, ray_d, far, fg_z, bg_z, batch['rgb'], depth_sup] + list(ret.values()):
                    if torch.is_tensor(t):
                        t.record_stream(stream)
                with torch.cuda.stream(stream):
                    eng.backward(g_rgb, g_depth, g_w, grad_scale=1.0 / self.world_size, out=self.grads[m][:L.LEVEL_PARAMS + 1], bad_count=self.bad_cameras,
                                 defer_reduce=True)
                    self._update_begin(m)
                scalars.append(sc)
                continue
            eng.backward(g_rgb, g_depth, g_w, grad_scale=1.0 / self.world_size, out=self.grads[m][:L.LEVEL_PARAMS + 1], bad_count=self.bad_cameras,
                         events=ev['bwd'] if ev else None, defer_reduce=True)
            scalars.append(sc)
            self._update_begin(m)
        return scalars


def batch_to_device(b, device):
    out = {}
    for k, v in b.items():
        if isinstance(v, np.ndarray):
            out[k] = torch.from_numpy(np.ascontiguousarray(v)).to(device)
    return out
```

Before: 496,700.

## Fuse composite forward, loss gradient and composite backward into one level-tail kernel

Adds a level_tail kernel that runs the volume-rendering composite forward, the loss head and the composite backward in one pass, writing d_out straight into the workspace. Forward and backward gain MLP-only entry points, so the separate composite kernels and the host-side loss/grad round trip are skipped on the default path. Loss scalars are now computed off the critical path on the update stream, and _update_end moves after fine sampling to widen overlap. The cost is a separate valid-depth-count pre-pass and more cross-stream event bookkeeping.

```diff
diff --git a/include/nerfpp_hip.h b/include/nerfpp_hip.h
--- a/include/nerfpp_hip.h
+++ b/include/nerfpp_hip.h
@@ -163,6 +163,43 @@
 
 int nerfpp_level_reduce_grads(void* stream, const nerfpp_backward_args* args);
 
+
+int nerfpp_valid_depth_count(void* stream, int n_rays, const float* depth_sup, float* n_valid);
+
+int nerfpp_level_forward_mlp(void* stream, const nerfpp_forward_args* args);
+
+typedef struct {
+  int32_t n_rays, n_samples;
+  int32_t precision;
+  int32_t loss_type;
+  float lambda_depth;
+  float kl_sigma;
+  const float* ray_d;
+  const float* fg_far;
+  const float* fg_z;
+  const float* bg_z;
+  void* workspace;
+  const float* rgb_gt;
+  const float* depth_sup;
+  const float* n_valid;
+  float* rgb;
+  float* depth;
+  float* fg_weights;
+  float* bg_weights;
+  float* fg_dists;
+  float* fg_rgb;
+  float* fg_depth;
+  float* bg_rgb;
+  float* bg_depth;
+  float* bg_lambda;
+} nerfpp_level_tail_args;
+
+int nerfpp_level_tail(void* stream, const nerfpp_level_tail_args* args);
+
+int nerfpp_level_backward_mlp(void* stream, const nerfpp_backward_args* args);
+
+int nerfpp_workspace_d_out(int n_rays, int n_samples, int precision, int net, int64_t* byte_offset);
+
 int nerfpp_adam_step(void* stream, float* params, const float* grads, float* exp_avg,
                      float* exp_avg_sq, int64_t n, int step, double lr, double beta1, double beta2,
                      double eps, const float* skip_if_nonzero);
diff --git a/outdoor_nerf_depth_amd/_lib.py b/outdoor_nerf_depth_amd/_lib.py
--- a/outdoor_nerf_depth_amd/_lib.py
+++ b/outdoor_nerf_depth_amd/_lib.py
@@ -42,6 +42,14 @@
                [(k, _fp) for k in ('rgb', 'depth', 'rgb_gt', 'depth_sup', 'bad_count')]
 
 
+class LevelTailArgs(C.Structure):
+    _fields_ = [('n_rays', C.c_int32), ('n_samples', C.c_int32), ('precision', C.c_int32), ('loss_type', C.c_int32),
+                ('lambda_depth', C.c_float), ('kl_sigma', C.c_float)] + \
+               [(k, _fp) for k in ('ray_d', 'fg_far', 'fg_z', 'bg_z', 'workspace', 'rgb_gt', 'depth_sup', 'n_valid',
+                                   'rgb', 'depth', 'fg_weights', 'bg_weights', 'fg_dists', 'fg_rgb', 'fg_depth', 'bg_rgb',
+                                   'bg_depth', 'bg_lambda')]
+
+
 SYMBOLS = {
     'nerfpp_last_error': (C.c_char_p, []),
     'nerfpp_abi_version': (C.c_int, []),
@@ -70,6 +78,11 @@
     'nerfpp_loss': (C.c_int, [_fp, C.c_int, C.c_int, C.c_int, C.c_float, C.c_float] + [_fp] * 12),
     'nerfpp_level_backward': (C.c_int, [_fp, C.POINTER(BackwardArgs)]),
     'nerfpp_level_reduce_grads': (C.c_int, [_fp, C.POINTER(BackwardArgs)]),
+    'nerfpp_valid_depth_count': (C.c_int, [_fp, C.c_int, _fp, _fp]),
+    'nerfpp_level_forward_mlp': (C.c_int, [_fp, C.POINTER(ForwardArgs)]),
+    'nerfpp_level_tail': (C.c_int, [_fp, C.POINTER(LevelTailArgs)]),
+    'nerfpp_level_backward_mlp': (C.c_int, [_fp, C.POINTER(BackwardArgs)]),
+    'nerfpp_workspace_d_out': (C.c_int, [C.c_int, C.c_int, C.c_int, C.c_int, _i64p]),
     'nerfpp_adam_step': (C.c_int, [_fp, _fp, _fp, _fp, _fp, C.c_int64, C.c_int, C.c_double, C.c_double,
                                    C.c_double, C.c_double, _fp]),
     'nerfpp_image_metrics_workspace_bytes': (C.c_int64, [C.c_int, C.c_int, C.c_int]),
diff --git a/outdoor_nerf_depth_amd/csrc/nerfpp_api.hip b/outdoor_nerf_depth_amd/csrc/nerfpp_api.hip
--- a/outdoor_nerf_depth_amd/csrc/nerfpp_api.hip
+++ b/outdoor_nerf_depth_amd/csrc/nerfpp_api.hip
@@ -1,5 +1,6 @@
 #include "probe_env.h"
 #include <hip/hip_runtime.h>
+#include <stddef.h>
 #include <stdio.h>
 #include <stdlib.h>
 #include <string.h>
@@ -281,13 +282,14 @@
   return NERFPP_OK;
 }
 
-int nerfpp_level_forward(void* stream, const nerfpp_forward_args* a) {
+static int level_forward(void* stream, const nerfpp_forward_args* a, bool composite) {
   REQUIRE(a, "args");
   REQUIRE(a->n_rays > 0 && a->n_samples >= 2 && a->n_samples <= NERFPP_MAX_SAMPLES, "sizes");
   REQUIRE(prec_ok_fwd(a->precision), "precision must be 1, 2 or 3");
   REQUIRE(a->ray_o && a->ray_d && a->fg_far && a->fg_z && a->bg_z && a->packed && a->workspace, "inputs");
-  REQUIRE(a->rgb && a->depth && a->fg_weights && a->bg_weights && a->fg_dists && a->fg_rgb && a->fg_depth &&
-          a->bg_rgb && a->bg_depth && a->bg_lambda, "outputs");
+  if (composite)
+    REQUIRE(a->rgb && a->depth && a->fg_weights && a->bg_weights && a->fg_dists && a->fg_rgb && a->fg_depth &&
+            a->bg_rgb && a->bg_depth && a->bg_lambda, "outputs");
   hipStream_t st = (hipStream_t)stream;
   const int P = a->precision;
   const bool train = a->training != 0;
@@ -322,11 +324,60 @@
     launch_mlp_fwd_pair(st, P, train, mm[0], mm[1], 0);
   }
   if (a->ev_mlp_end) (void)hipEventRecord((hipEvent_t)a->ev_mlp_end, st);
-  launch_composite_fwd(st, a->n_rays, a->n_samples, (const float*)(ws + L.out_raw[0]),
-                       (const float*)(ws + L.out_raw[1]), (const float*)(ws + L.depth_real), a->ray_d, a->fg_far,
-                       a->fg_z, a->bg_z, a->rgb, a->depth, a->fg_weights, a->bg_weights, a->fg_dists, a->fg_rgb,
-                       a->fg_depth, a->bg_rgb, a->bg_depth, a->bg_lambda);
-  return check_launch("level_forward");
+  if (composite)
+    launch_composite_fwd(st, a->n_rays, a->n_samples, (const float*)(ws + L.out_raw[0]),
+                         (const float*)(ws + L.out_raw[1]), (const float*)(ws + L.depth_real), a->ray_d, a->fg_far,
+                         a->fg_z, a->bg_z, a->rgb, a->depth, a->fg_weights, a->bg_weights, a->fg_dists, a->fg_rgb,
+                         a->fg_depth, a->bg_rgb, a->bg_depth, a->bg_lambda);
+  return check_launch(composite ? "level_forward" : "level_forward_mlp");
+}
+int nerfpp_level_forward(void* stream, const nerfpp_forward_args* a) { return level_forward(stream, a, true); }
+int nerfpp_level_forward_mlp(void* stream, const nerfpp_forward_args* a) { return level_forward(stream, a, false); }
+
+static_assert(sizeof(nerfpp_level_tail_args) == 168, "nerfpp_level_tail_args: size");
+static_assert(offsetof(nerfpp_level_tail_args, loss_type) == 12, "nerfpp_level_tail_args: loss_type");
+static_assert(offsetof(nerfpp_level_tail_args, kl_sigma) == 20, "nerfpp_level_tail_args: kl_sigma");
+static_assert(offsetof(nerfpp_level_tail_args, ray_d) == 24, "nerfpp_level_tail_args: ray_d");
+static_assert(offsetof(nerfpp_level_tail_args, workspace) == 56, "nerfpp_level_tail_args: workspace");
+static_assert(offsetof(nerfpp_level_tail_args, n_valid) == 80, "nerfpp_level_tail_args: n_valid");
+static_assert(offsetof(nerfpp_level_tail_args, rgb) == 88, "nerfpp_level_tail_args: rgb");
+static_assert(offsetof(nerfpp_level_tail_args, bg_lambda) == 160, "nerfpp_level_tail_args: bg_lambda");
+
+int nerfpp_valid_depth_count(void* stream, int n_rays, const float* depth_sup, float* n_valid) {
+  REQUIRE(n_rays > 0 && depth_sup && n_valid, "n_rays > 0, non-null pointers");
+  launch_valid_depth_count((hipStream_t)stream, n_rays, depth_sup, n_valid);
+  return check_launch("valid_depth_count");
+}
+
+int nerfpp_level_tail(void* stream, const nerfpp_level_tail_args* a) {
+  REQUIRE(a, "args");
+  REQUIRE(a->n_rays > 0 && a->n_samples >= 2 && a->n_samples <= NERFPP_MAX_SAMPLES, "sizes");
+  REQUIRE(prec_ok_fwd(a->precision), "precision must be 1, 2 or 3");
+  REQUIRE(a->ray_d && a->fg_far && a->fg_z && a->bg_z && a->workspace, "inputs");
+  REQUIRE(a->rgb && a->depth && a->fg_weights && a->bg_weights && a->fg_dists && a->fg_rgb && a->fg_depth &&
+          a->bg_rgb && a->bg_depth && a->bg_lambda, "outputs");
+  REQUIRE(a->loss_type >= NERFPP_LOSS_RGB_ONLY && a->loss_type <= NERFPP_LOSS_KL, "loss_type in 0..3");
+  REQUIRE(a->rgb_gt, "rgb_gt");
+  if (a->loss_type != NERFPP_LOSS_RGB_ONLY) REQUIRE(a->depth_sup, "a depth loss needs depth_sup");
+  if (a->loss_type == NERFPP_LOSS_MSE || a->loss_type == NERFPP_LOSS_L1) REQUIRE(a->n_valid, "mse / l1 need n_valid (nerfpp_valid_depth_count)");
+  if (a->loss_type == NERFPP_LOSS_KL) REQUIRE(a->kl_sigma > 0.f, "kl_sigma > 0");
+  const WsLayout L = ws_layout(a->n_rays, a->n_samples, a->precision, true);
+  char* ws = (char*)a->workspace;
+  TailLoss tl{};
+  tl.type = a->loss_type; tl.lambda_depth = a->lambda_depth; tl.kl_sigma = a->kl_sigma;
+  tl.rgb_gt = a->rgb_gt; tl.depth_sup = a->depth_sup; tl.n_valid = a->n_valid;
+  launch_level_tail((hipStream_t)stream, a->n_rays, a->n_samples, (const float*)(ws + L.out_raw[0]),
+                    (const float*)(ws + L.out_raw[1]), (const float*)(ws + L.depth_real), a->ray_d, a->fg_far, a->fg_z,
+                    a->bg_z, a->rgb, a->depth, a->fg_weights, a->bg_weights, a->fg_dists, a->fg_rgb, a->fg_depth,
+                    a->bg_rgb, a->bg_depth, a->bg_lambda, (float*)(ws + L.d_out[0]), (float*)(ws + L.d_out[1]), tl);
+  return check_launch("level_tail");
+}
+
+int nerfpp_workspace_d_out(int n_rays, int n_samples, int precision, int net, int64_t* byte_offset) {
+  REQUIRE(n_rays > 0 && n_samples >= 2 && n_samples <= NERFPP_MAX_SAMPLES && prec_ok_fwd(precision), "sizes / precision");
+  REQUIRE(net >= 0 && net < N_NET && byte_offset, "net / non-null output");
+  *byte_offset = (int64_t)ws_layout(n_rays, n_samples, precision, true).d_out[net];
+  return NERFPP_OK;
 }
 
 int nerfpp_loss(void* stream, int n_rays, int n_samples, int loss_type, float lambda_depth, float kl_sigma,
@@ -405,21 +456,23 @@
   return check_launch("level_reduce_grads");
 }
 
-int nerfpp_level_backward(void* stream, const nerfpp_backward_args* a) {
+}
+
+static int level_backward(void* stream, const nerfpp_backward_args* a, bool composite) {
   REQUIRE(a, "args");
   REQUIRE(a->n_rays > 0 && a->n_samples >= 2 && a->n_samples <= NERFPP_MAX_SAMPLES, "sizes");
   REQUIRE(prec_ok(a->precision), "precision must be 1 or 2");
   REQUIRE(a->ray_d && a->fg_far && a->fg_z && a->bg_z && a->packed && a->workspace && a->tables, "inputs");
   REQUIRE(a->grads && a->params, "gradients / params");
   LossFuse lf{};
-  if (a->fused_loss) {
+  if (composite && a->fused_loss) {
     REQUIRE(a->loss_type >= NERFPP_LOSS_RGB_ONLY && a->loss_type <= NERFPP_LOSS_KL, "loss_type in 0..3");
     REQUIRE(a->rgb && a->rgb_gt, "fused loss head needs rgb and rgb_gt");
     if (a->loss_type != NERFPP_LOSS_RGB_ONLY) REQUIRE(a->depth && a->depth_sup, "fused depth loss needs depth and depth_sup");
     if (a->loss_type == NERFPP_LOSS_KL) REQUIRE(a->kl_sigma > 0.f, "kl_sigma > 0");
     lf.type = a->loss_type; lf.lambda_depth = a->lambda_depth; lf.kl_sigma = a->kl_sigma;
     lf.rgb = a->rgb; lf.depth = a->depth; lf.rgb_gt = a->rgb_gt; lf.depth_sup = a->depth_sup;
-  } else {
+  } else if (composite) {
     REQUIRE(a->g_rgb && a->g_depth, "dL/d rgb and dL/d depth (or fused_loss)");
   }
   hipStream_t st = (hipStream_t)stream;
@@ -431,10 +484,11 @@
   const TblLayout T = tbl_layout();
   char* ws = (char*)a->workspace;
   const char* pk = (const char*)a->packed;
-  launch_composite_bwd(st, a->n_rays, a->n_samples, (const float*)(ws + L.out_raw[0]),
-                       (const float*)(ws + L.out_raw[1]), (const float*)(ws + L.depth_real), a->ray_d, a->fg_far,
-                       a->fg_z, a->bg_z, a->g_rgb, a->g_depth, a->g_fg_weights, (float*)(ws + L.d_out[0]),
-                       (float*)(ws + L.d_out[1]), a->fused_loss ? &lf : nullptr);
+  if (composite)
+    launch_composite_bwd(st, a->n_rays, a->n_samples, (const float*)(ws + L.out_raw[0]),
+                         (const float*)(ws + L.out_raw[1]), (const float*)(ws + L.depth_real), a->ray_d, a->fg_far,
+                         a->fg_z, a->bg_z, a->g_rgb, a->g_depth, a->g_fg_weights, (float*)(ws + L.d_out[0]),
+                         (float*)(ws + L.d_out[1]), a->fused_loss ? &lf : nullptr);
   MlpBwdArgs mb[N_NET];
   for (int net = 0; net < N_NET; ++net) {
     MlpBwdArgs& m = mb[net];
@@ -457,8 +511,13 @@
   if (a->ev_bwd_end) (void)hipEventRecord((hipEvent_t)a->ev_bwd_end, st);
   if (!(a->defer_reduce && defer_dw())) weight_grads(st, a, L);
   if (!a->defer_reduce) reduce_grads(st, a, L, T);
-  return check_launch("level_backward");
-}
+  return check_launch(composite ? "level_backward" : "level_backward_mlp");
+}
+
+extern "C" {
+
+int nerfpp_level_backward(void* stream, const nerfpp_backward_args* a) { return level_backward(stream, a, true); }
+int nerfpp_level_backward_mlp(void* stream, const nerfpp_backward_args* a) { return level_backward(stream, a, false); }
 
 int nerfpp_adam_step(void* stream, float* params, const float* grads, float* exp_avg, float* exp_avg_sq,
                      int64_t n, int step, double lr, double beta1, double beta2, double eps,
diff --git a/outdoor_nerf_depth_amd/csrc/nerfpp_kernels.h b/outdoor_nerf_depth_amd/csrc/nerfpp_kernels.h
--- a/outdoor_nerf_depth_amd/csrc/nerfpp_kernels.h
+++ b/outdoor_nerf_depth_amd/csrc/nerfpp_kernels.h
@@ -47,6 +47,14 @@
   const float* depth_sup;
 };
 
+struct TailLoss {
+  int type;
+  float lambda_depth, kl_sigma;
+  const float* rgb_gt;
+  const float* depth_sup;
+  const float* n_valid;
+};
+
 struct DwArgs {
   NetWs ws[N_NET];
   int64_t rows, rows_padded;
@@ -81,6 +89,12 @@
                           const float* depth_real_bg, const float* ray_d, const float* fg_far,
                           const float* fg_z, const float* bg_z, const float* g_rgb, const float* g_depth,
                           const float* g_fg_weights, float* dout_fg, float* dout_bg, const nerfpp::LossFuse* lf);
+void launch_level_tail(hipStream_t st, int n, int S, const float* raw_fg, const float* raw_bg,
+                       const float* depth_real_bg, const float* ray_d, const float* fg_far, const float* fg_z,
+                       const float* bg_z, float* rgb, float* depth, float* fg_weights, float* bg_weights,
+                       float* fg_dists, float* fg_rgb, float* fg_depth, float* bg_rgb, float* bg_depth,
+                       float* bg_lambda, float* dout_fg, float* dout_bg, const nerfpp::TailLoss& tl);
+void launch_valid_depth_count(hipStream_t st, int n, const float* depth_sup, float* n_valid);
 void launch_loss(hipStream_t st, int n, int S, int type, float lambda_depth, float kl_sigma, const float* rgb,
                  const float* rgb_gt, const float* depth, const float* depth_sup, const float* fg_weights,
                  const float* fg_z, const float* fg_dists, const float* fg_far, float* scalars, float* g_rgb,
diff --git a/outdoor_nerf_depth_amd/csrc/nerfpp_render.hip b/outdoor_nerf_depth_amd/csrc/nerfpp_render.hip
--- a/outdoor_nerf_depth_amd/csrc/nerfpp_render.hip
+++ b/outdoor_nerf_depth_amd/csrc/nerfpp_render.hip
@@ -322,14 +322,44 @@
   }
 }
 
+template <bool BG>
+__device__ __forceinline__ void volume_forward(const RaySamples& v, int S, int cpl, int lane, size_t row0,
+                                               float* __restrict__ weights, float* __restrict__ dists, float sums[4]) {
+  float a0 = 0, a1 = 0, a2 = 0, ad = 0;
+#pragma unroll
+  for (int k = 0; k < CPL_MAX; ++k) {
+    const int i = lane * cpl + k;
+    if (k < cpl && i < S) {
+      weights[row0 + i] = v.w[k];
+      if (!BG) dists[row0 + i] = v.dist[k];
+      a0 += v.w[k] * v.c[k][0]; a1 += v.w[k] * v.c[k][1]; a2 += v.w[k] * v.c[k][2];
+      ad += v.w[k] * v.zval[k];
+    }
+  }
+  sums[0] = wave_sum(a0); sums[1] = wave_sum(a1); sums[2] = wave_sum(a2); sums[3] = wave_sum(ad);
+}
+
+struct CompositeOut {
+  float *rgb, *depth, *fg_rgb, *fg_depth, *bg_rgb, *bg_depth, *bg_lambda;
+};
+__device__ __forceinline__ void composite_store(const CompositeOut& o, int ray, int lane, const float f[4], const float b[4],
+                                                float lam, float rgb_depth[4]) {
+  const float b0 = lam * b[0], b1 = lam * b[1], b2 = lam * b[2];
+  const float bd = lam * b[3];
+  rgb_depth[0] = f[0] + b0; rgb_depth[1] = f[1] + b1; rgb_depth[2] = f[2] + b2; rgb_depth[3] = f[3] + bd;
+  if (lane == 0) {
+    o.fg_rgb[ray * 3] = f[0]; o.fg_rgb[ray * 3 + 1] = f[1]; o.fg_rgb[ray * 3 + 2] = f[2];
+    o.bg_rgb[ray * 3] = b0; o.bg_rgb[ray * 3 + 1] = b1; o.bg_rgb[ray * 3 + 2] = b2;
+    o.rgb[ray * 3] = rgb_depth[0]; o.rgb[ray * 3 + 1] = rgb_depth[1]; o.rgb[ray * 3 + 2] = rgb_depth[2];
+    o.fg_depth[ray] = f[3]; o.bg_depth[ray] = bd; o.depth[ray] = rgb_depth[3]; o.bg_lambda[ray] = lam;
+  }
+}
+
 __global__ __launch_bounds__(256) void composite_fwd_kernel(
     int n, int S, const float4* __restrict__ raw_fg, const float4* __restrict__ raw_bg,
     const float* __restrict__ depth_real_bg, const float* __restrict__ ray_d,
     const float* __restrict__ fg_far, const float* __restrict__ fg_z, const float* __restrict__ bg_z,
-    float* __restrict__ rgb, float* __restrict__ depth, float* __restrict__ fg_weights,
-    float* __restrict__ bg_weights, float* __restrict__ fg_dists, float* __restrict__ fg_rgb,
-    float* __restrict__ fg_depth, float* __restrict__ bg_rgb, float* __restrict__ bg_depth,
-    float* __restrict__ bg_lambda) {
+    float* __restrict__ fg_weights, float* __restrict__ bg_weights, float* __restrict__ fg_dists, CompositeOut out) {
   const int wave = threadIdx.x >> 6, lane = threadIdx.x & 63;
   const int ray = blockIdx.x * 4 + wave;
   if (ray >= n) return;
@@ -338,39 +368,13 @@
   const float dx = ray_d[ray * 3], dy = ray_d[ray * 3 + 1], dz = ray_d[ray * 3 + 2];
   const float dnorm = sqrtf(sum3(dx * dx, dy * dy, dz * dz));
   RaySamples v;
+  float f[4], b[4], rgb_depth[4];
   load_volume<false>(v, S, cpl, lane, row0, raw_fg, fg_z + row0, nullptr, dnorm, fg_far[ray]);
-  float a0 = 0, a1 = 0, a2 = 0, ad = 0;
-#pragma unroll
-  for (int k = 0; k < CPL_MAX; ++k) {
-    const int i = lane * cpl + k;
-    if (k < cpl && i < S) {
-      fg_weights[row0 + i] = v.w[k];
-      fg_dists[row0 + i] = v.dist[k];
-      a0 += v.w[k] * v.c[k][0]; a1 += v.w[k] * v.c[k][1]; a2 += v.w[k] * v.c[k][2];
-      ad += v.w[k] * v.zval[k];
-    }
-  }
-  const float f0 = wave_sum(a0), f1 = wave_sum(a1), f2 = wave_sum(a2), fd = wave_sum(ad);
+  volume_forward<false>(v, S, cpl, lane, row0, fg_weights, fg_dists, f);
   const float lam = v.lambda;
   load_volume<true>(v, S, cpl, lane, row0, raw_bg, bg_z + row0, depth_real_bg, dnorm, 0.f);
-  a0 = a1 = a2 = ad = 0;
-#pragma unroll
-  for (int k = 0; k < CPL_MAX; ++k) {
-    const int i = lane * cpl + k;
-    if (k < cpl && i < S) {
-      bg_weights[row0 + i] = v.w[k];
-      a0 += v.w[k] * v.c[k][0]; a1 += v.w[k] * v.c[k][1]; a2 += v.w[k] * v.c[k][2];
-      ad += v.w[k] * v.zval[k];
-    }
-  }
-  const float b0 = lam * wave_sum(a0), b1 = lam * wave_sum(a1), b2 = lam * wave_sum(a2);
-  const float bd = lam * wave_sum(ad);
-  if (lane == 0) {
-    fg_rgb[ray * 3] = f0; fg_rgb[ray * 3 + 1] = f1; fg_rgb[ray * 3 + 2] = f2;
-    bg_rgb[ray * 3] = b0; bg_rgb[ray * 3 + 1] = b1; bg_rgb[ray * 3 + 2] = b2;
-    rgb[ray * 3] = f0 + b0; rgb[ray * 3 + 1] = f1 + b1; rgb[ray * 3 + 2] = f2 + b2;
-    fg_depth[ray] = fd; bg_depth[ray] = bd; depth[ray] = fd + bd; bg_lambda[ray] = lam;
-  }
+  volume_forward<true>(v, S, cpl, lane, row0, bg_weights, nullptr, b);
+  composite_store(out, ray, lane, f, b, lam, rgb_depth);
 }
 
 struct KlFuse { bool on; float gt, inv2s, lambda_depth; };
@@ -415,6 +419,29 @@
   }
 }
 
+__device__ __forceinline__ void loss_head_grad(int type, float lambda_depth, float kl_sigma, int n, int ray,
+                                               const float rgb_depth[4], const float* __restrict__ rgb_gt,
+                                               const float* __restrict__ depth_sup, const float* __restrict__ fg_far,
+                                               float cnt, float gC[3], float& gD, KlFuse& kl) {
+#pragma unroll
+  for (int c = 0; c < 3; ++c) gC[c] = 2.f * (rgb_depth[c] - rgb_gt[ray * 3 + c]) / (float)(3 * n);
+  gD = 0.f;
+  if (type == 1 || type == 2) {
+    const float gt = depth_sup[ray];
+    if (gt > 0.f && cnt > 0.f) {
+      const float d = rgb_depth[3] - gt;
+      gD = type == 1 ? lambda_depth * 2.f * d / cnt
+                     : lambda_depth * (d > 0.f ? 1.f : (d < 0.f ? -1.f : 0.f)) / cnt;
+    }
+  } else if (type == 3) {
+    const float gt = depth_sup[ray];
+    kl.on = gt > 0.f && gt < fg_far[ray];
+    kl.gt = gt;
+    kl.inv2s = 1.f / (2.f * kl_sigma);
+    kl.lambda_depth = lambda_depth;
+  }
+}
+
 template <bool LF>
 __global__ __launch_bounds__(256) void composite_bwd_kernel(
     int n, int S, const float4* __restrict__ raw_fg, const float4* __restrict__ raw_bg,
@@ -442,23 +469,8 @@
   float gC[3], gD;
   KlFuse kl{false, 0.f, 0.f, 0.f};
   if (LF) {
-#pragma unroll
-    for (int c = 0; c < 3; ++c) gC[c] = 2.f * (lf.rgb[ray * 3 + c] - lf.rgb_gt[ray * 3 + c]) / (float)(3 * n);
-    gD = 0.f;
-    if (lf.type == 1 || lf.type == 2) {
-      const float gt = lf.depth_sup[ray];
-      if (gt > 0.f && cnt > 0.f) {
-        const float d = lf.depth[ray] - gt;
-        gD = lf.type == 1 ? lf.lambda_depth * 2.f * d / cnt
-                          : lf.lambda_depth * (d > 0.f ? 1.f : (d < 0.f ? -1.f : 0.f)) / cnt;
-      }
-    } else if (lf.type == 3) {
-      const float gt = lf.depth_sup[ray];
-      kl.on = gt > 0.f && gt < fg_far[ray];
-      kl.gt = gt;
-      kl.inv2s = 1.f / (2.f * lf.kl_sigma);
-      kl.lambda_depth = lf.lambda_depth;
-    }
+    const float rgb_depth[4] = {lf.rgb[ray * 3], lf.rgb[ray * 3 + 1], lf.rgb[ray * 3 + 2], lf.depth ? lf.depth[ray] : 0.f};
+    loss_head_grad(lf.type, lf.lambda_depth, lf.kl_sigma, n, ray, rgb_depth, lf.rgb_gt, lf.depth_sup, fg_far, cnt, gC, gD, kl);
   } else {
     gC[0] = g_rgb[ray * 3]; gC[1] = g_rgb[ray * 3 + 1]; gC[2] = g_rgb[ray * 3 + 2];
     gD = g_depth[ray];
@@ -478,6 +490,48 @@
   volume_backward<false>(vf, S, cpl, lane, row0, gC, gD, g_lam * lam, LF ? nullptr : g_fg_weights, dout_fg, kl);
   const float gCb[3] = {lam * gC[0], lam * gC[1], lam * gC[2]};
   volume_backward<true>(vb, S, cpl, lane, row0, gCb, lam * gD, 0.f, nullptr, dout_bg);
+}
+
+__global__ __launch_bounds__(256) void level_tail_kernel(
+    int n, int S, const float4* __restrict__ raw_fg, const float4* __restrict__ raw_bg,
+    const float* __restrict__ depth_real_bg, const float* __restrict__ ray_d,
+    const float* __restrict__ fg_far, const float* __restrict__ fg_z, const float* __restrict__ bg_z,
+    float* __restrict__ fg_weights, float* __restrict__ bg_weights, float* __restrict__ fg_dists, CompositeOut out,
+    float4* __restrict__ dout_fg, float4* __restrict__ dout_bg, TailLoss tl) {
+  const int wave = threadIdx.x >> 6, lane = threadIdx.x & 63;
+  const int ray = blockIdx.x * 4 + wave;
+  if (ray >= n) return;
+  const int cpl = (S + 63) / 64;
+  const size_t row0 = (size_t)ray * S;
+  const float dx = ray_d[ray * 3], dy = ray_d[ray * 3 + 1], dz = ray_d[ray * 3 + 2];
+  const float dnorm = sqrtf(sum3(dx * dx, dy * dy, dz * dz));
+  RaySamples vf, vb;
+  float f[4], b[4], rgb_depth[4];
+  load_volume<false>(vf, S, cpl, lane, row0, raw_fg, fg_z + row0, nullptr, dnorm, fg_far[ray]);
+  volume_forward<false>(vf, S, cpl, lane, row0, fg_weights, fg_dists, f);
+  const float lam = vf.lambda;
+  load_volume<true>(vb, S, cpl, lane, row0, raw_bg, bg_z + row0, depth_real_bg, dnorm, 0.f);
+  volume_forward<true>(vb, S, cpl, lane, row0, bg_weights, nullptr, b);
+  composite_store(out, ray, lane, f, b, lam, rgb_depth);
+  float gC[3], gD;
+  KlFuse kl{false, 0.f, 0.f, 0.f};
+  const float cnt = (tl.type == 1 || tl.type == 2) ? tl.n_valid[0] : 0.f;
+  loss_head_grad(tl.type, tl.lambda_depth, tl.kl_sigma, n, ray, rgb_depth, tl.rgb_gt, tl.depth_sup, fg_far, cnt, gC, gD, kl);
+  const float g_lam = gC[0] * b[0] + gC[1] * b[1] + gC[2] * b[2] + gD * b[3];
+  volume_backward<false>(vf, S, cpl, lane, row0, gC, gD, g_lam * lam, nullptr, dout_fg, kl);
+  const float gCb[3] = {lam * gC[0], lam * gC[1], lam * gC[2]};
+  volume_backward<true>(vb, S, cpl, lane, row0, gCb, lam * gD, 0.f, nullptr, dout_bg);
+}
+
+__global__ __launch_bounds__(256) void valid_depth_count_kernel(int n, const float* __restrict__ depth_sup,
+                                                                float* __restrict__ n_valid) {
+  __shared__ int s_cnt[4];
+  int c = 0;
+  for (int r = threadIdx.x; r < n; r += 256) c += depth_sup[r] > 0.f ? 1 : 0;
+  c = wave_sum(c);
+  if ((threadIdx.x & 63) == 0) s_cnt[threadIdx.x >> 6] = c;
+  __syncthreads();
+  if (threadIdx.x == 0) n_valid[0] = (float)((s_cnt[0] + s_cnt[1]) + (s_cnt[2] + s_cnt[3]));
 }
 
 __device__ double block_sum(double v, double* sh) {
@@ -621,8 +675,21 @@
                           float* bg_weights, float* fg_dists, float* fg_rgb, float* fg_depth, float* bg_rgb,
                           float* bg_depth, float* bg_lambda) {
   hipLaunchKernelGGL(composite_fwd_kernel, dim3((n + 3) / 4), dim3(256), 0, st, n, S, (const float4*)raw_fg,
-                     (const float4*)raw_bg, depth_real_bg, ray_d, fg_far, fg_z, bg_z, rgb, depth, fg_weights,
-                     bg_weights, fg_dists, fg_rgb, fg_depth, bg_rgb, bg_depth, bg_lambda);
+                     (const float4*)raw_bg, depth_real_bg, ray_d, fg_far, fg_z, bg_z, fg_weights, bg_weights, fg_dists,
+                     CompositeOut{rgb, depth, fg_rgb, fg_depth, bg_rgb, bg_depth, bg_lambda});
+}
+void launch_level_tail(hipStream_t st, int n, int S, const float* raw_fg, const float* raw_bg,
+                       const float* depth_real_bg, const float* ray_d, const float* fg_far, const float* fg_z,
+                       const float* bg_z, float* rgb, float* depth, float* fg_weights, float* bg_weights,
+                       float* fg_dists, float* fg_rgb, float* fg_depth, float* bg_rgb, float* bg_depth,
+                       float* bg_lambda, float* dout_fg, float* dout_bg, const nerfpp::TailLoss& tl) {
+  hipLaunchKernelGGL(level_tail_kernel, dim3((n + 3) / 4), dim3(256), 0, st, n, S, (const float4*)raw_fg,
+                     (const float4*)raw_bg, depth_real_bg, ray_d, fg_far, fg_z, bg_z, fg_weights, bg_weights, fg_dists,
+                     CompositeOut{rgb, depth, fg_rgb, fg_depth, bg_rgb, bg_depth, bg_lambda}, (float4*)dout_fg,
+                     (float4*)dout_bg, tl);
+}
+void launch_valid_depth_count(hipStream_t st, int n, const float* depth_sup, float* n_valid) {
+  hipLaunchKernelGGL(valid_depth_count_kernel, dim3(1), dim3(256), 0, st, n, depth_sup, n_valid);
 }
 void launch_composite_bwd(hipStream_t st, int n, int S, const float* raw_fg, const float* raw_bg,
                           const float* depth_real_bg, const float* ray_d, const float* fg_far,
diff --git a/outdoor_nerf_depth_amd/ops.py b/outdoor_nerf_depth_amd/ops.py
--- a/outdoor_nerf_depth_amd/ops.py
+++ b/outdoor_nerf_depth_amd/ops.py
@@ -198,7 +198,9 @@
             self.workspace = torch.empty(need, dtype=torch.uint8, device=self.device)
         return self.workspace
 
-    def forward(self, ray_o, ray_d, fg_z_max, fg_z_vals, bg_z_vals, training=False, events=None):
+    def forward(self, ray_o, ray_d, fg_z_max, fg_z_vals, bg_z_vals, training=False, events=None, composite=True):
+        if not composite and not training:
+            raise L.NerfppError('forward(composite=False) is the first part of a training level (level_tail follows)')
         ray_o, ray_d = _f32(ray_o), _f32(ray_d)
         n = ray_o.shape[0]
         fg_z_vals = _f32(fg_z_vals)
@@ -221,10 +223,43 @@
             setattr(a, k, out[k].data_ptr())
         if events is not None:
             a.ev_mlp_begin, a.ev_mlp_end = events[0].cuda_event, events[1].cuda_event
-        L.check(L.lib().nerfpp_level_forward(_stream(), C.byref(a)), 'nerfpp_level_forward')
+        if composite:
+            L.check(L.lib().nerfpp_level_forward(_stream(), C.byref(a)), 'nerfpp_level_forward')
+        else:
+            L.check(L.lib().nerfpp_level_forward_mlp(_stream(), C.byref(a)), 'nerfpp_level_forward_mlp')
         if training:
             self._fwd = (n, S, ray_d, fg_z_max, fg_z_vals, bg_z_vals)
         return out
+
+    def level_tail(self, ret, rgb_gt, depth_sup=None, loss_type='rgbonly', lambda_depth=1.0, kl_sigma=0.01, n_valid=None):
+        if self._fwd is None:
+            raise L.NerfppError('level_tail() needs a preceding forward(training=True, composite=False)')
+        n, S, ray_d, fg_far, fg_z, bg_z = self._fwd
+        t = L.LOSS_TYPES[loss_type]
+        rgb_gt = _f32(rgb_gt, (n, 3))
+        depth_sup = _f32(depth_sup, (n,)) if t != L.LOSS_RGB_ONLY else None
+        if t in (L.LOSS_MSE, L.LOSS_L1):
+            if n_valid is None or n_valid.dtype != torch.float32 or n_valid.numel() != 1 or n_valid.device != self.device:
+                raise L.NerfppError('level_tail(): mse / l1 need n_valid = valid_depth_count(depth_sup)')
+        a = L.LevelTailArgs()
+        a.n_rays, a.n_samples, a.precision, a.loss_type = n, S, self.precision, t
+        a.lambda_depth, a.kl_sigma = float(lambda_depth), float(kl_sigma)
+        a.ray_d, a.fg_far, a.fg_z, a.bg_z = [x.data_ptr() for x in (ray_d, fg_far, fg_z, bg_z)]
+        a.workspace = self.workspace.data_ptr()
+        a.rgb_gt, a.depth_sup, a.n_valid = _p(rgb_gt), _p(depth_sup), _p(n_valid)
+        for k in RET_KEYS:
+            shape = (n, 3) if k in ('rgb', 'fg_rgb', 'bg_rgb') else (n, S) if k in ('fg_weights', 'bg_weights', 'fg_dists') else (n,)
+            setattr(a, k, _f32(ret[k], shape).data_ptr())
+        L.check(L.lib().nerfpp_level_tail(_stream(), C.byref(a)), 'nerfpp_level_tail')
+        return ret
+
+    def d_out(self, net):
+        if self._fwd is None:
+            raise L.NerfppError('d_out() needs a preceding forward(training=True)')
+        n, S = self._fwd[0], self._fwd[1]
+        off = C.c_int64()
+        L.check(L.lib().nerfpp_workspace_d_out(n, S, self.precision, int(net), C.byref(off)), 'nerfpp_workspace_d_out')
+        return self.workspace[off.value: off.value + n * S * 16].view(torch.float32).view(n * S, 4)
 
     def saved_tensor(self, net, tensor, plane=0):
         if self._fwd is None:
@@ -242,12 +277,15 @@
         return blk.reshape(rows_p, ld)[:rows].float()
 
     def backward(self, g_rgb, g_depth, g_fg_weights=None, grad_scale=1.0, out=None, events=None, defer_reduce=False,
-                 fused_loss=None, bad_count=None):
+                 fused_loss=None, bad_count=None, from_tail=False):
         if self._fwd is None:
             raise L.NerfppError('backward() needs a preceding forward(training=True)')
         n, S, ray_d, fg_far, fg_z, bg_z = self._fwd
         keep = None
-        if fused_loss is None:
+        if from_tail:
+            if fused_loss is not None or g_rgb is not None or g_depth is not None or g_fg_weights is not None:
+                raise L.NerfppError('backward(from_tail=True) takes no upstream gradients: level_tail() formed them')
+        elif fused_loss is None:
             g_rgb, g_depth = _f32(g_rgb, (n, 3)), _f32(g_depth, (n,))
             g_fg_weights = _f32(g_fg_weights, (n, S)) if g_fg_weights is not None else None
         else:
@@ -265,10 +303,10 @@
         a.workspace_precision = self.precision
         a.ray_d, a.fg_far, a.fg_z, a.bg_z = [t.data_ptr() for t in (ray_d, fg_far, fg_z, bg_z)]
         a.packed, a.workspace, a.tables = self.packed_bwd.data_ptr(), self.workspace.data_ptr(), self.tables.data_ptr()
-        if fused_loss is None:
+        if fused_loss is None and not from_tail:
             a.g_rgb, a.g_depth = g_rgb.data_ptr(), g_depth.data_ptr()
             a.g_fg_weights = g_fg_weights.data_ptr() if g_fg_weights is not None else None
-        else:
+        elif fused_loss is not None:
             a.fused_loss, a.loss_type = 1, t
             a.lambda_depth, a.kl_sigma = float(fused_loss.get('lambda_depth', 1.0)), float(fused_loss.get('kl_sigma', 0.01))
             a.rgb, a.depth, a.rgb_gt = keep[0].data_ptr(), keep[1].data_ptr(), keep[2].data_ptr()
@@ -283,7 +321,10 @@
             if bad_count.dtype != torch.int32 or bad_count.numel() != 1 or bad_count.device != self.device:
                 raise L.NerfppError('bad_count: one int32 on the engine\'s device')
             a.bad_count = bad_count.data_ptr()
-        L.check(L.lib().nerfpp_level_backward(_stream(), C.byref(a)), 'nerfpp_level_backward')
+        if from_tail:
+            L.check(L.lib().nerfpp_level_backward_mlp(_stream(), C.byref(a)), 'nerfpp_level_backward_mlp')
+        else:
+            L.check(L.lib().nerfpp_level_backward(_stream(), C.byref(a)), 'nerfpp_level_backward')
         self._bwd_args = (a, grads, bad_count, torch.cuda.current_stream()) if defer_reduce else None
         return grads
 
@@ -321,6 +362,13 @@
     return scalars, g_rgb, g_depth, g_w
 
 
+def valid_depth_count(depth_sup):
+    depth_sup = _f32(depth_sup)
+    out = torch.empty(1, device=depth_sup.device)
+    L.check(L.lib().nerfpp_valid_depth_count(_stream(), depth_sup.numel(), _p(depth_sup), _p(out)), 'nerfpp_valid_depth_count')
+    return out
+
+
 def adam_step(params, grads, exp_avg, exp_avg_sq, step, lr=5e-4, beta1=0.9, beta2=0.999, eps=1e-8, skip=None):
     if skip is not None and (skip.dtype != torch.float32 or not skip.is_cuda):
         raise L.NerfppError('adam_step: skip must be a float32 device tensor')
diff --git a/outdoor_nerf_depth_amd/trainer.py b/outdoor_nerf_depth_amd/trainer.py
--- a/outdoor_nerf_depth_amd/trainer.py
+++ b/outdoor_nerf_depth_amd/trainer.py
@@ -1,3 +1,4 @@
+import functools
 import os
 
 import numpy as np
@@ -17,7 +18,7 @@
     def __init__(self, device, precision=L.PREC_SPLIT_BF16, cascade_samples=(64, 128), lrate=5e-4,
                  use_depth=True, depth_loss_type='mse', lambda_depth=0.1, depth_sigma=0.01, depth_scale=1.0,
                  world_size=1, level_params=None, overlap_allreduce=True, optim_autoexpo=False, img_names=None,
-                 lambda_autoexpo=1.0, seed=777, torch_rng=False, fuse_loss=False, comm=None):
+                 lambda_autoexpo=1.0, seed=777, torch_rng=False, fuse_loss=False, comm=None, level_tail=True):
         self.device = torch.device(device)
         self.comm = comm
         self.precision = precision
@@ -39,6 +40,8 @@
         self.step_count = 0
         self.seed, self.torch_rng = int(seed), bool(torch_rng)
         self.fuse_loss = bool(fuse_loss)
+        self.level_tail = bool(level_tail)
+        self._loss_ready = []
         self.rng_step = 0
         self.bad_cameras = torch.zeros(1, dtype=torch.int32, device=self.device)
         self.autoexpo = None
@@ -89,20 +92,28 @@
             self.autoexpo[m].apply(self._ae_grad[m][:, :2], self._ae_grad[m][:, 2] > 0)
             self._ae_grad[m] = None
 
-    def _update_begin(self, m):
+    def _update_begin(self, m, loss=None):
         if self.update_stream is None:
+            sc = loss() if loss is not None else None
             self._update(m, self.step_count)
-            return
+            return sc
         ev = torch.cuda.Event()
         ev.record()
         self.update_stream.wait_event(ev)
         if self._ae_grad[m] is not None:
             self._ae_grad[m].record_stream(self.update_stream)
+        sc = None
         with torch.cuda.stream(self.update_stream):
+            if loss is not None:
+                sc = loss()
+                ready = torch.cuda.Event()
+                ready.record()
+                self._loss_ready.append(ready)
             self._update(m, self.step_count)
             done = torch.cuda.Event()
             done.record()
         self._pending[m] = done
+        return sc
 
     def _update_end(self, m):
         done = self._pending.pop(m, None)
@@ -150,6 +161,7 @@
                                                 bad=self.bad_cameras)
         depth_sup = batch.get('depth_sup') if self.loss_type != 'rgbonly' else None
         scalars = []
+        keep = []
         ret = None
         ae_idx = None
         if self.autoexpo is not None:
@@ -157,8 +169,9 @@
             if name is None and 'frame' in batch:
                 name = self.img_names[int(batch['frame'])]
             ae_idx = self.autoexpo[0].lookup(name)
+        tail = self.level_tail and not self.fuse_loss and ae_idx is None and events is None
+        n_valid = ops.valid_depth_count(depth_sup) if tail and self.loss_type in ('mse', 'l1') else None
         for m, eng in enumerate(self.engines):
-            self._update_end(m)
             if m > 0 and rng is not None:
                 fg_z, bg_z = ops.sample_fine_pair(fg_z, ret['fg_weights'], bg_z, ret['bg_weights'], S1, rng=rng)
             elif m > 0:
@@ -167,9 +180,29 @@
                 fg_z, bg_z = ops.sample_fine_pair(fg_z, ret['fg_weights'], bg_z, ret['bg_weights'], S1,
                                                   u_fg=u_fg, u_bg=u_bg)
             ev = events[m] if events is not None else None
+            self._update_end(m)
             ret = eng.forward(ray_o, ray_d, far, fg_z, bg_z, training=True,
-                              events=ev['fwd'] if ev else None)
+                              events=ev['fwd'] if ev else None, composite=not tail)
             ae = self.autoexpo[m] if ae_idx is not None else None
+            if tail:
+                eng.level_tail(ret, batch['rgb'], depth_sup, self.loss_type, self.lambda_depth, self.kl_sigma, n_valid=n_valid)
+                loss = functools.partial(self._scalars, ret, batch['rgb'], depth_sup, fg_z, far)
+                keep.append((ret, fg_z, far))
+                bwd = dict(grad_scale=1.0 / self.world_size, out=self.grads[m][:L.LEVEL_PARAMS + 1], bad_count=self.bad_cameras,
+                           defer_reduce=True, from_tail=True)
+                if self.concurrent_backward and m + 1 < len(self.engines) and self.update_stream is not None:
+                    stream = self.level_streams[m]
+                    fwd_done = torch.cuda.Event()
+                    fwd_done.record()
+                    stream.wait_event(fwd_done)
+                    with torch.cuda.stream(stream):
+                        eng.backward(None, None, None, **bwd)
+                        scalars.append(self._update_begin(m, loss))
+                else:
+                    eng.backward(None, None, None, **bwd)
+                    scalars.append(loss())
+                    self._update_begin(m)
+                continue
             if ae is None and self.fuse_loss:
                 loss_done = None
                 if self.update_stream is not None:
@@ -221,7 +254,13 @@
                          events=ev['bwd'] if ev else None, defer_reduce=True)
             scalars.append(sc)
             self._update_begin(m)
+        for ready in self._loss_ready:
+            torch.cuda.current_stream().wait_event(ready)
+        del self._loss_ready[:]
         return scalars
+
+    def _scalars(self, ret, rgb_gt, depth_sup, fg_z, far):
+        return ops.loss_and_grads(ret, rgb_gt, depth_sup, self.loss_type, self.lambda_depth, self.kl_sigma, fg_z, far)[0]
 
 
 def batch_to_device(b, device):
```

After: 496,000. About the same (-0.1%).
